# lms-org/trajectory_controller

Measured on AMD Instinct MI355X. Metric: MPC QP solves/sec (horizon N=20, 2 inputs) at 1/2/4/8 MI355X; max|du| vs dlib, higher is better.
Workload: dtype f64; 1 GPU; batch 262144 trajectories per GPU, N=20, 2 inputs, compact (mpcControllerTobi) form, cold start, eps 0.01, max_iter 10000; global_batch=262144, horizon=20, algo=lane_fma, parallelism=batch-sharded x1, batches_in_flight=1, gather=none (1 GPU)

## Files before the change

### trajectory_controller_amd/capi.py

```python
from __future__ import annotations

import ctypes as C
import os

_HERE = os.path.dirname(os.path.abspath(__file__))
LIB_PATH = os.environ.get("TPC_MPC_LIB") or os.path.join(_HERE, "lib", "libtpc_mpc.so")

OK = 0
F64, F32 = 0, 1
HOST, DEVICE = 0, 1
ALGO_AUTO, ALGO_WAVE, ALGO_LANE, ALGO_LANE_FMA, ALGO_GROUP = 0, 1, 2, 3, 4
OPT_WAVE_GROUP, OPT_MAILBOX_HOST, OPT_GROUP_LANES, OPT_HOST_SOLVE_ONE = 1, 2, 3, 4
DEVICE_NONE = -1
FLAG_NONFINITE, FLAG_MAX_ITER, FLAG_BAD_MODEL, FLAG_NOT_POLISHED = 0x1, 0x2, 0x4, 0x8
NEWTON_FALLBACK_SOLVE, NEWTON_FALLBACK_NONE = 0, 1
NEWTON_FALLBACKS = {"solve": NEWTON_FALLBACK_SOLVE, "none": NEWTON_FALLBACK_NONE}
LOOP_RECORD, LOOP_POLISHED, LOOP_NEWTON = 0, 1, 2
PARAM_FAST_CAPPED = 0x1

STATUS_NAMES = {0: "OK", 1: "BAD_ARG", 2: "BAD_WEIGHTS", 3: "BAD_BOUNDS", 4: "BAD_HORIZON",
                5: "BAD_EPS", 6: "NO_DEVICE", 7: "HIP", 8: "ALLOC", 9: "COMM"}
ABI_VERSION = 5
COMM_ID_BYTES = 128

# ... 99 lines not shown
            f"(python -c 'import __graft_entry__ as g; g.build()' or make -C trajectory_controller_amd/csrc)")
    try:
        import torch
    except ImportError:
        pass
    lib = C.CDLL(path)
    vp, i32p, u32p = C.c_void_p, C.POINTER(C.c_int32), C.POINTER(C.c_uint32)
    lib.tpc_mpc_abi_version.restype = C.c_int
    lib.tpc_mpc_supported_horizons.argtypes = [C.POINTER(C.c_int), C.c_int]
    lib.tpc_mpc_default_params.argtypes = [C.POINTER(Params), C.c_int]
    lib.tpc_mpc_create.argtypes = [C.c_int, C.POINTER(vp)]
    lib.tpc_mpc_destroy.argtypes = [vp]
    lib.tpc_mpc_last_error.argtypes = [vp]
    lib.tpc_mpc_last_error.restype = C.c_char_p
    lib.tpc_mpc_solve_one.argtypes = [vp, C.POINTER(Params), C.c_double, C.c_double, C.c_double,
                                      C.POINTER(C.c_double), C.POINTER(C.c_double)]
    lib.tpc_mpc_last_flags.argtypes = [vp, u32p, i32p]
    lib.tpc_mpc_solve_batch_compact.argtypes = [vp, C.POINTER(Params), C.c_int64, vp, vp, vp, vp, vp,
                                                vp, u32p, C.c_int, vp]
    lib.tpc_mpc_solve_batch_general.argtypes = [vp, C.POINTER(Params), C.POINTER(GeneralIO), u32p,
                                                C.c_int, vp]
    lib.tpc_mpc_solve_batch_general_backward.argtypes = [vp, C.POINTER(Params), C.POINTER(GeneralIO),
                                                         C.POINTER(GeneralGrad), u32p, C.c_int, vp]
    lib.tpc_mpc_polish_batch_general.argtypes = [vp, C.POINTER(Params), C.POINTER(GeneralIO), C.POINTER(Polish), u32p,
                                                 C.c_int, vp]
    lib.tpc_mpc_solve_batch_general_sharded.argtypes = [vp, C.POINTER(Params), C.POINTER(GeneralIO), u32p, vp]
    lib.tpc_mpc_rollout.argtypes = [vp, C.POINTER(Params), C.POINTER(GeneralIO), C.c_int32, vp, vp, vp,
                                    vp, u32p, C.c_int, vp]
    lib.tpc_mpc_rollout_record.argtypes = [vp, C.POINTER(Params), C.POINTER(GeneralIO), C.c_int32, vp, vp, vp,
                                           vp, vp, u32p, C.c_int, vp]
    lib.tpc_mpc_rollout_polished.argtypes = [vp, C.POINTER(Params), C.POINTER(GeneralIO), C.c_int32, vp,
                                             C.POINTER(Polish), vp, vp, vp, vp, u32p, C.c_int, vp]
    lib.tpc_mpc_rollout_newton.argtypes = [vp, C.POINTER(Params), C.POINTER(GeneralIO), C.c_int32, vp,
                                           C.POINTER(Polish), C.c_int32, vp, vp, vp, vp, vp, u32p, C.c_int, vp]
    lib.tpc_mpc_rollout_backward.argtypes = [vp, C.POINTER(Params), C.POINTER(GeneralIO), C.c_int32, vp,
                                             C.POINTER(RolloutGrad), u32p, C.c_int, vp]
    lib.tpc_mpc_solve_batch_general_forward.argtypes = [vp, C.POINTER(Params), C.POINTER(GeneralIO), vp,
                                                        C.POINTER(Tangents), vp, u32p, C.c_int, vp]
    lib.tpc_mpc_rollout_forward.argtypes = [vp, C.POINTER(Params), C.POINTER(GeneralIO), C.c_int32, vp, vp, vp,
                                            C.POINTER(Tangents), vp, vp, u32p, C.c_int, vp]
    lib.tpc_mpc_rollout_plant.argtypes = [vp, C.POINTER(Params), C.POINTER(GeneralIO), C.POINTER(Plant), C.c_int32,
                                          C.c_int32, vp, C.POINTER(Polish), C.c_int32, vp, vp, vp, vp, vp, u32p,
                                          C.c_int, vp]
    lib.tpc_mpc_rollout_plant_backward.argtypes = [vp, C.POINTER(Params), C.POINTER(GeneralIO), C.POINTER(Plant),
                                                   C.c_int32, vp, C.POINTER(RolloutGrad), C.POINTER(PlantGrad), u32p,
                                                   C.c_int, vp]
    lib.tpc_mpc_rollout_plant_forward.argtypes = [vp, C.POINTER(Params), C.POINTER(GeneralIO), C.POINTER(Plant),
                                                  C.c_int32, vp, vp, vp, C.POINTER(Tangents),
                                                  C.POINTER(PlantTangents), vp, vp, u32p, C.c_int, vp]
    lib.tpc_mpc_set_profiling.argtypes = [vp, C.c_int]
    lib.tpc_mpc_last_kernel_times.argtypes = [vp, C.POINTER(C.c_double), C.POINTER(C.c_double),
                                              C.POINTER(C.c_int)]
    lib.tpc_mpc_follow_batch.argtypes = [vp, C.POINTER(Params), C.POINTER(Trajectories), vp, vp, C.c_int32,
                                         vp, vp, vp, vp, vp, u32p, vp]
    lib.tpc_mpc_last_lane_stats.argtypes = [vp, C.POINTER(C.c_uint64), C.POINTER(C.c_uint64)]
    lib.tpc_mpc_x_set_work_hint.argtypes = [vp, vp, C.c_int64, C.c_int]
    lib.tpc_mpc_set_option.argtypes = [vp, C.c_int, C.c_int64]
    lib.tpc_mpc_x_set_group_share.argtypes = [vp, C.c_int, C.c_int]
    lib.tpc_mpc_x_set_lanex_below.argtypes = [vp, C.c_int64]
    lib.tpc_mpc_x_set_queue_key.argtypes = [vp, C.c_int]
    lib.tpc_mpc_x_last_queue_key.argtypes = [vp, C.POINTER(C.c_int)]
    lib.tpc_mpc_x_queue_key_predict.argtypes = [vp, vp, vp, C.c_int64, vp]
    lib.tpc_mpc_gather_shards.argtypes = [vp, C.c_int64, C.POINTER(C.c_void_p), C.c_int, C.c_int, vp]
    lib.tpc_mpc_reserve.argtypes = [vp, C.POINTER(Params), C.c_int64, C.c_int]
    lib.tpc_mpc_build_info.restype = C.c_char_p
    lib.tpc_mpc_set_resident.argtypes = [vp, C.c_int64]
    lib.tpc_mpc_solve_batch_compact_mixed.argtypes = [vp, C.POINTER(Params), C.c_int64, vp, vp, vp, vp, vp, vp,
                                                      vp, u32p, C.c_int, vp]
    lib.tpc_mpc_follow_batch_horizon.argtypes = [vp, C.POINTER(Params), C.POINTER(Trajectories), vp, vp, vp,
                                                 C.c_int32, vp, vp, vp, vp, vp, vp, u32p, vp]
    lib.tpc_mpc_comm_unique_id.argtypes = [vp, C.c_size_t]
    lib.tpc_mpc_comm_init_rank.argtypes = [vp, vp, C.c_size_t, C.c_int, C.c_int]
    lib.tpc_mpc_comm_test_mode.argtypes = [vp, C.c_int, C.c_int]
    lib.tpc_mpc_comm_destroy.argtypes = [vp]
    lib.tpc_mpc_shard_range.argtypes = [C.c_int64, C.c_int, C.c_int, C.POINTER(C.c_int64), C.POINTER(C.c_int64)]
    lib.tpc_mpc_solve_batch_compact_sharded.argtypes = [vp, C.POINTER(Params), C.c_int64, vp, vp, vp, vp, vp, vp,
                                                        u32p, vp]
    i64p = C.POINTER(C.c_int64)
    lib.tpc_mpc_shard_map.argtypes = [C.c_int64, C.c_int, C.c_int, C.c_int, i64p, i64p, i64p]
    lib.tpc_mpc_solve_batch_compact_sharded_split.argtypes = [vp, C.POINTER(Params), C.c_int64, C.c_int, vp, vp, vp, vp, vp, vp,
                                                              u32p, vp]
    lib.tpc_mpc_gather_shards_split.argtypes = [vp, C.c_int64, C.c_int, C.POINTER(C.c_void_p), C.c_int, C.c_int, vp]
    lib.tpc_mpc_x_exchange_plan.argtypes = [C.c_int64, C.c_int, C.c_int, C.c_int, C.c_int, i64p, C.c_int, i64p]
    for name in EXPORTS:
        getattr(lib, name)
    if path == LIB_PATH:
        _lib = lib
    return lib


def default_params(horizon: int, dtype: int = F64, algo: int = ALGO_AUTO, **overrides) -> Params:
    lib = load_library()
    p = Params()
    rc = lib.tpc_mpc_default_params(C.byref(p), horizon)
    if rc != OK:
        raise TpcMpcError(rc, f"unsupported horizon {horizon}")
    p.dtype, p.algo = dtype, algo
    for k, val in overrides.items():
        if k in ("lower", "upper"):
            getattr(p, k)[0], getattr(p, k)[1] = float(val[0]), float(val[1])
        else:
            setattr(p, k, val)
    return p
```

### trajectory_controller_amd/csrc/mpc_internal.h

```cpp
#pragma once

#include <hip/hip_runtime.h>
#include <stdint.h>

namespace tpc {

constexpr int kWave = 64;

struct Knobs {
    double eps;
    uint32_t max_iter;
    uint32_t smo_iters;
};

struct CompactArgs {
    int64_t n;
    const void *v, *dy, *dphi;
    void *front, *rear;
    int32_t* iters;
    uint32_t* flags;
    const int32_t* work_hint;
    double step, wheelbase;
    double q[2], r[2], lo[2], hi[2];
    int table_key;
};

constexpr int kQueueKeyLambda = 0, kQueueKeyTableUsed = 1, kQueueKeyHint = 2;

struct OneArgs {
    double v, dy, dphi;
    double step, wheelbase;
    double q[2], r[2], lo[2], hi[2];
    uint64_t* out;
    uint64_t* info;
    static constexpr int32_t* iters = nullptr;
    static constexpr uint32_t* flags = nullptr;
};

struct GeneralArgs {
    int64_t n, ld;
    const void *A, *B, *C, *Q, *R, *lo, *hi, *x0, *targets;
    void *controls, *v;
    void* u0;
    int32_t* iters;
    uint32_t* flags;
    const int32_t* work_hint;
    int shift_controls;
};

struct Workspace {
    void* state;
    uint32_t* ticket;
    unsigned long long* stats;
    int64_t capacity_bytes;
    uint32_t *keys, *rank, *order;
    void* sort_temp;
    size_t sort_temp_bytes;
    hipEvent_t* ev;
    int wave_group = 0;
    int group_lanes = 0;
    int max_waves = 0;
    bool group_pair = false;
    int64_t lanex_below = -1;
    int cu_count = 0;
};

constexpr int kQueueTickets = 16;
constexpr int kQueueTicketStride = 64;
constexpr int64_t kQueueTicketBytes = (int64_t)kQueueTickets * kQueueTicketStride * 4;
constexpr int64_t kWaveQueueMaxInstances = 32768;

constexpr int kAlgoMixed = 101;
constexpr int kAlgoGeneric = 100;
constexpr int kMaxHorizon = 64;
int64_t generic_scratch_bytes(int H, int dtype, int64_t n);
hipError_t generic_compact(int dtype, int H, const CompactArgs& a, const Knobs& k, void* scratch, hipStream_t s);
hipError_t generic_general(int dtype, int I, int H, const GeneralArgs& a, const Knobs& k, void* scratch, hipStream_t s);

size_t sort_temp_bytes(int64_t n);
hipError_t order_begin(void* temp, hipStream_t s);
hipError_t presolve_merge(const uint32_t* queue, const uint32_t* queue_len, int64_t n, const void* sf, const void* sr,
                          const int32_t* si, void* f, void* r, int32_t* it, uint32_t limit, hipStream_t s);
hipError_t presolve_merge_rows(const uint32_t* queue, const uint32_t* queue_len, int64_t n, const void* su, const int32_t* si,
                               void* u, int32_t* it, int rows, int64_t ld, uint32_t limit, hipStream_t s);
const uint32_t* order_queue_len(const void* temp);
hipError_t order_finish(const uint32_t* keys, const uint32_t* rank, uint32_t* order, int64_t n, void* temp,
                        hipStream_t s);

struct RolloutStepArgs {
    int64_t n, ld, ld_out, ld_nlt;
    int I, H, step, steps;
    const void *A, *B, *C;
    void* x;
    void* targets;
    const void* controls;
    const void* new_last_targets;
    void* controls_out;
    void* states_out;
    const int32_t* iters_step;
    int32_t* iters_out;
    void* sequences_out;
    const void* disturbance;
    int64_t ld_d;
};
hipError_t launch_rollout_step(int dtype, const RolloutStepArgs& a, hipStream_t s);

struct FollowArgs {
    int64_t n, ld;
    int max_points;
    const float *px, *py, *dx, *dy, *vel;
    const int32_t* count;
    const float* car_velocity;
    const float* look_ahead;
    const float *lut_x, *lut_y;
    int lut_n;
    double *v_out, *ysoll_out, *phisoll_out;
    float *target_speed, *target_distance;
};
hipError_t launch_traj_point(const FollowArgs& a, hipStream_t s);
struct FollowHorizonArgs {
    int H;
    int64_t ldw;
    const float* step_spacing;
    double step, wheelbase;
    double q[2], r[2], lo[2], hi[2];
    double *A, *B, *C, *Q, *R, *lo_out, *hi_out, *x0, *targets;
    double* targets_copy;
    int64_t ld_copy;
};
hipError_t launch_traj_horizon(const FollowArgs& a, const FollowHorizonArgs& f, hipStream_t s);
hipError_t launch_follow_post(int64_t n, const float* target_speed, double* front, double* rear, hipStream_t s);

}
```

### trajectory_controller_amd/csrc/mpc_lane_inst.hip

```cpp
#include <cstdint>

#include "mpc_lane.h"
#include "mpc_lanex.h"

#ifndef TPC_LANE_H
#error "compile with -DTPC_LANE_H=<horizon>"
#endif

namespace tpc {

namespace {

constexpr int kH = TPC_LANE_H;

template <class Tag, class Kernel>
inline int pg_grid(Kernel kernel, int block) {
    constexpr int kMaxDev = 64;
    static int cache[kMaxDev] = {0};
    int dev = 0;
    if (hipGetDevice(&dev) != hipSuccess) dev = 0;
    if (dev >= 0 && dev < kMaxDev && cache[dev] > 0) return cache[dev];
    int cus = 256, per_cu = 4;
    hipDeviceProp_t prop;
    if (hipGetDeviceProperties(&prop, dev) == hipSuccess) cus = prop.multiProcessorCount;
    if (hipOccupancyMaxActiveBlocksPerMultiprocessor(&per_cu, kernel, block, 0) != hipSuccess || per_cu < 1)
        per_cu = 1;
    if (per_cu > 4) per_cu = 4;
    if (dev >= 0 && dev < kMaxDev) cache[dev] = cus * per_cu;
    return cus * per_cu;
}
struct TagState {}; struct TagFast {}; struct TagExact {}; struct TagLanex {}; template <int I> struct TagLanexG {};

inline bool wants_state(const CompactArgs&) { return false; }
inline bool wants_state(const GeneralArgs& a) { return a.controls != nullptr || a.v != nullptr; }

template <typename T, int I, class Model, class Args>
hipError_t phase1(const Args& a, const Knobs& k, const Workspace& ws, hipStream_t s) {
    T* recs = (T*)ws.state;
    hipError_t e = hipMemsetAsync(ws.ticket, 0, sizeof(uint32_t), s);
    if (e == hipSuccess) e = hipMemsetAsync(ws.stats, 0, 3 * sizeof(unsigned long long), s);
    if (e == hipSuccess) e = order_begin(ws.sort_temp, s);
    if (e != hipSuccess) return e;
    const int cd_grid = (int)((a.n + kWave - 1) / kWave);
    if (ws.ev) (void)hipEventRecord(ws.ev[0], s);
    hipLaunchKernelGGL((lane_cd_kernel<T, I, kH, Model, Args>), dim3(cd_grid), dim3(kWave), 0, s, a, k, recs,
                       ws.keys, ws.rank, (uint32_t*)ws.sort_temp, ws.stats, wants_state(a) ? 0 : 1);
    e = hipGetLastError();
    if (e != hipSuccess) return e;
    e = order_finish(ws.keys, ws.rank, ws.order, a.n, ws.sort_temp, s);
    if (e != hipSuccess) return e;
    if (ws.ev) (void)hipEventRecord(ws.ev[1], s);
    return hipSuccess;
}
template <typename T, int I, class Model, class Args>
hipError_t phase2(const Args& a, const Knobs& k, const Workspace& ws, hipStream_t s, bool only_if_refused) {
    T* recs = (T*)ws.state;
    if (wants_state(a)) {
        const int grid_cap = pg_grid<TagState>(lane_pg_kernel<T, I, kH, Model, Args>, kWave);
        const int64_t need = (a.n + kWave - 1) / kWave;
        hipLaunchKernelGGL((lane_pg_kernel<T, I, kH, Model, Args>), dim3((unsigned)(need < grid_cap ? need : grid_cap)),
                           dim3(kWave), 0, s, a, k, (const T*)recs, (const uint32_t*)ws.order, ws.ticket, ws.stats,
                           only_if_refused ? 1 : 0);
    } else {
        constexpr int bt = kWave * FusedOcc<T, kH>::value;
        const int64_t need = (a.n + bt - 1) / bt;
        const uint32_t* queue_len = order_queue_len(ws.sort_temp);
        if constexpr (Model::kFastStop) {
            if (!only_if_refused) {
                const int fast_cap = pg_grid<TagFast>(lane_pg_fused_kernel<T, I, kH, Model, Args, true>, bt);
                hipLaunchKernelGGL((lane_pg_fused_kernel<T, I, kH, Model, Args, true>),
                                   dim3((unsigned)(need < fast_cap ? need : fast_cap)), dim3(bt), 0, s, a, k,
                                   (const T*)recs, (const uint32_t*)ws.order, ws.ticket, ws.stats, queue_len);
            }
        }
        const int grid_cap = pg_grid<TagExact>(lane_pg_fused_kernel<T, I, kH, Model, Args, false>, bt);
        hipLaunchKernelGGL((lane_pg_fused_kernel<T, I, kH, Model, Args, false>),
                           dim3((unsigned)(need < grid_cap ? need : grid_cap)), dim3(bt), 0, s, a, k,
                           (const T*)recs, (const uint32_t*)ws.order, ws.ticket, ws.stats, queue_len);
    }
    return hipGetLastError();
}

inline int64_t lanex_below(const Workspace& ws, bool general) {
    if (ws.lanex_below >= 0) return ws.lanex_below;
    const int64_t at = general ? (kH == 40 ? 49152 : (kH == 30 ? 57344 : (kH == 20 ? 81920 : (kH == 10 ? 98304 : 0))))
                               : (kH == 40 ? 60000 : (kH == 30 ? 65536 : (kH == 20 || kH == 10 ? 98304 : 0)));
    const int cus = ws.cu_count > 0 ? ws.cu_count : 256;
    return at * cus / 256 < at ? at * cus / 256 : at;
}

template <typename T, int I, class Model, class Args>
hipError_t run(const Args& a, const Knobs& k, const Workspace& ws, hipStream_t s) {
    if (a.n <= 0) return hipSuccess;
    hipError_t e = phase1<T, I, Model, Args>(a, k, ws, s);
    if (e != hipSuccess) return e;
    if constexpr (std::is_same<Model, CompactModel<T>>::value && sizeof(T) == 8 && LanexPlan<kH>::built) {
        if (a.n < lanex_below(ws, false)) {
            constexpr int ng = LanexPlan<kH>::NG;
            const int64_t need = (a.n + ng - 1) / ng;
            const int grid_cap = pg_grid<TagLanex>(lanex_pg_kernel<T, kH>, kWave);
            hipLaunchKernelGGL((lanex_pg_kernel<T, kH>), dim3((unsigned)(need < grid_cap ? need : grid_cap)), dim3(kWave), 0, s, a, k,
                               (const T*)ws.state, (const uint32_t*)ws.order, ws.ticket, ws.stats, order_queue_len(ws.sort_temp),
                               GroupRefillBatch<LanexPlan<kH>::G>::value);
            e = hipGetLastError();
            if (ws.ev) (void)hipEventRecord(ws.ev[2], s);
            return e;
        }
    }
    if constexpr (std::is_same<Args, GeneralArgs>::value && sizeof(T) == 8 && LanexPlan<kH>::built) {
        if (a.n < lanex_below(ws, true)) {
            constexpr int ng = LanexPlan<kH>::NG;
            const int64_t need = (a.n + ng - 1) / ng;
            if (wants_state(a)) {
                const int grid_cap = pg_grid<TagLanexG<I + 2>>(lanexg_pg_kernel<T, I, kH, true>, kWave);
                hipLaunchKernelGGL((lanexg_pg_kernel<T, I, kH, true>), dim3((unsigned)(need < grid_cap ? need : grid_cap)), dim3(kWave), 0, s,
                                   a, k, (const T*)ws.state, (const uint32_t*)ws.order, ws.ticket, ws.stats, (const uint32_t*)nullptr,
                                   GroupRefillBatch<LanexPlan<kH>::G>::value);
            } else {
                const int grid_cap = pg_grid<TagLanexG<I>>(lanexg_pg_kernel<T, I, kH>, kWave);
                hipLaunchKernelGGL((lanexg_pg_kernel<T, I, kH>), dim3((unsigned)(need < grid_cap ? need : grid_cap)), dim3(kWave), 0, s, a, k,
                                   (const T*)ws.state, (const uint32_t*)ws.order, ws.ticket, ws.stats, order_queue_len(ws.sort_temp),
                                   GroupRefillBatch<LanexPlan<kH>::G>::value);
            }
            e = hipGetLastError();
            if (ws.ev) (void)hipEventRecord(ws.ev[2], s);
            return e;
        }
    }
    e = phase2<T, I, Model, Args>(a, k, ws, s, false);
    if (ws.ev) (void)hipEventRecord(ws.ev[2], s);
    return e;
}

template <typename T, int I, class Model, class Args, int SUBSET = 1>
hipError_t resolve(const Args& a, const Knobs& k, const Workspace& ws, const int32_t* select, const uint32_t* gate, hipStream_t s,
                   double lambda_from = 0.0, const uint32_t* pre_len = nullptr, uint32_t pre_limit = 0u) {
    if (a.n <= 0) return hipSuccess;
    T* recs = (T*)ws.state;
    uint32_t* queue_len = ws.ticket + 1;
    hipError_t e = hipMemsetAsync(ws.ticket, 0, 32, s);
    if (e != hipSuccess) return e;
    const int grid = (int)((a.n + kWave - 1) / kWave);
    hipLaunchKernelGGL((lane_cd_kernel<T, I, kH, Model, Args, SUBSET>), dim3(grid), dim3(kWave), 0, s, a, k, recs, ws.order,
                       (uint32_t*)nullptr, queue_len, ws.stats, 1, select, gate, (T)lambda_from, pre_len, pre_limit);
    if constexpr (std::is_same<Model, CompactModel<T>>::value && sizeof(T) == 8 && LanexPlan<kH>::built) {
        constexpr int ng = LanexPlan<kH>::NG;
        const int64_t need = (a.n + ng - 1) / ng;
        if constexpr (SUBSET == 2) {
            const int64_t solo = (int64_t)pre_limit / ng;
            hipLaunchKernelGGL((lanex_pg_kernel<T, kH, true>), dim3((unsigned)(need < solo ? need : solo)), dim3(kWave), 0, s, a, k,
                               (const T*)recs, (const uint32_t*)ws.order, ws.ticket, ws.stats, (const uint32_t*)queue_len, 1, pre_limit);
            return hipGetLastError();
        }
        const int grid_cap = pg_grid<TagLanex>(lanex_pg_kernel<T, kH>, kWave);
        hipLaunchKernelGGL((lanex_pg_kernel<T, kH>), dim3((unsigned)(need < grid_cap ? need : grid_cap)), dim3(kWave), 0, s, a, k,
                           (const T*)recs, (const uint32_t*)ws.order, ws.ticket, ws.stats, (const uint32_t*)queue_len, 1);
        return hipGetLastError();
    } else if constexpr (std::is_same<Args, GeneralArgs>::value && sizeof(T) == 8 && LanexPlan<kH>::built) {
        constexpr int ng = LanexPlan<kH>::NG;
        const int64_t need = (a.n + ng - 1) / ng;
        if constexpr (SUBSET == 2) {
            const int64_t solo = (int64_t)pre_limit / ng;
            hipLaunchKernelGGL((lanexg_pg_kernel<T, I, kH, false, true>), dim3((unsigned)(need < solo ? need : solo)), dim3(kWave), 0, s,
                               a, k, (const T*)recs, (const uint32_t*)ws.order, ws.ticket, ws.stats, (const uint32_t*)queue_len, 1, pre_limit);
            return hipGetLastError();
        }
        const int grid_cap = pg_grid<TagLanexG<I>>(lanexg_pg_kernel<T, I, kH>, kWave);
        hipLaunchKernelGGL((lanexg_pg_kernel<T, I, kH>), dim3((unsigned)(need < grid_cap ? need : grid_cap)), dim3(kWave), 0, s, a, k,
                           (const T*)recs, (const uint32_t*)ws.order, ws.ticket, ws.stats, (const uint32_t*)queue_len, 1);
        return hipGetLastError();
    } else {
    constexpr int bt = kWave * FusedOcc<T, kH>::value;
    const int64_t need = (a.n + bt - 1) / bt;
    const int grid_cap = pg_grid<TagExact>(lane_pg_fused_kernel<T, I, kH, Model, Args, false>, bt);
    hipLaunchKernelGGL((lane_pg_fused_kernel<T, I, kH, Model, Args, false>), dim3((unsigned)(need < grid_cap ? need : grid_cap)),
                       dim3(bt), 0, s, a, k, (const T*)recs, (const uint32_t*)ws.order, ws.ticket, ws.stats, (const uint32_t*)queue_len);
    return hipGetLastError();
    }
}

}

#define TPC_CAT2(a, b) a##b
#define TPC_CAT(a, b) TPC_CAT2(a, b)

#ifndef TPC_SCHED_NAME
#define TPC_SCHED_NAME "default"
#endif
const char* TPC_CAT(lane_build_h, TPC_LANE_H)() { return "sched=" TPC_SCHED_NAME; }

int64_t TPC_CAT(lane_rec_len_h, TPC_LANE_H)(int dtype) {
    return dtype == 0 ? LaneRec<double, kH>::kLen : LaneRec<float, kH>::kLen;
}

hipError_t TPC_CAT(lane_compact_h, TPC_LANE_H)(int dtype, const CompactArgs& a, const Knobs& k,
                                                 const Workspace& ws, hipStream_t s) {
    if (dtype == 0) return run<double, 2, CompactModel<double>, CompactArgs>(a, k, ws, s);
    return run<float, 2, CompactModel<float>, CompactArgs>(a, k, ws, s);
}

hipError_t TPC_CAT(lane_resolve_compact_h, TPC_LANE_H)(const CompactArgs& a, const Knobs& k, const Workspace& ws,
                                                         const int32_t* select, const uint32_t* gate, hipStream_t s,
                                                         double presolved_from, const uint32_t* pre_len, uint32_t pre_limit) {
    return resolve<double, 2, CompactModel<double>, CompactArgs>(a, k, ws, select, gate, s, presolved_from, pre_len, pre_limit);
}
hipError_t TPC_CAT(lane_presolve_compact_h, TPC_LANE_H)(const CompactArgs& a, const Knobs& k, const Workspace& ws,
                                                          double lambda_from, uint32_t limit, hipStream_t s) {
    if constexpr (!LanexPlan<kH>::built) return hipErrorInvalidValue;
    return resolve<double, 2, CompactModel<double>, CompactArgs, 2>(a, k, ws, nullptr, nullptr, s, lambda_from, nullptr, limit);
}
hipError_t TPC_CAT(lane_resolve_general_h, TPC_LANE_H)(int I, const GeneralArgs& a, const Knobs& k, const Workspace& ws,
                                                         const int32_t* select, const uint32_t* gate, hipStream_t s,
                                                         double presolved_from, const uint32_t* pre_len, uint32_t pre_limit) {
    if (I == 2) return resolve<double, 2, GeneralModel<double, 2>, GeneralArgs>(a, k, ws, select, gate, s, presolved_from, pre_len, pre_limit);
    return resolve<double, 1, GeneralModel<double, 1>, GeneralArgs>(a, k, ws, select, gate, s, presolved_from, pre_len, pre_limit);
}
hipError_t TPC_CAT(lane_presolve_general_h, TPC_LANE_H)(int I, const GeneralArgs& a, const Knobs& k, const Workspace& ws,
                                                          double lambda_from, uint32_t limit, hipStream_t s) {
    if constexpr (!LanexPlan<kH>::built) return hipErrorInvalidValue;
    if (I == 2) return resolve<double, 2, GeneralModel<double, 2>, GeneralArgs, 2>(a, k, ws, nullptr, nullptr, s, lambda_from, nullptr, limit);
    return resolve<double, 1, GeneralModel<double, 1>, GeneralArgs, 2>(a, k, ws, nullptr, nullptr, s, lambda_from, nullptr, limit);
}

// ... 21 lines not shown
```

### trajectory_controller_amd/csrc/mpc_sort.hip

```cpp
#include "mpc_internal.h"

namespace tpc {

namespace {

constexpr int kBins = 1 << 16;

constexpr int kScanBlocks = 64, kScanThreads = 256, kPerThread = kBins / kScanBlocks / kScanThreads;

__global__ __launch_bounds__(kScanThreads) void scan_sums_kernel(const uint32_t* __restrict__ hist,
                                                                 uint32_t* __restrict__ block_sum) {
    __shared__ uint32_t part[kScanThreads / 64];
    const int t = threadIdx.x;
    const int top = kBins - 1 - (blockIdx.x * kScanThreads + t) * kPerThread;
    uint32_t sum = 0;
    for (int j = 0; j < kPerThread; ++j) sum += hist[top - j];
    for (int off = 32; off > 0; off >>= 1) sum += __shfl_down(sum, off);
    if ((t & 63) == 0) part[t >> 6] = sum;
    __syncthreads();
    if (t == 0) {
        uint32_t tot = 0;
        for (int w = 0; w < kScanThreads / 64; ++w) tot += part[w];
        block_sum[blockIdx.x] = tot;
    }
}

__global__ __launch_bounds__(kScanThreads) void scan_apply_kernel(uint32_t* __restrict__ hist,
                                                                  const uint32_t* __restrict__ block_sum) {
    __shared__ uint32_t part[kScanThreads];
    const int t = threadIdx.x;
    const int top = kBins - 1 - (blockIdx.x * kScanThreads + t) * kPerThread;
    uint32_t c[kPerThread], sum = 0;
    for (int j = 0; j < kPerThread; ++j) { c[j] = hist[top - j]; sum += c[j]; }
    part[t] = sum;
    __syncthreads();
    for (int off = 1; off < kScanThreads; off <<= 1) {
        const uint32_t add = t >= off ? part[t - off] : 0u;
        __syncthreads();
        part[t] += add;
        __syncthreads();
    }
    uint32_t base = part[t] - sum;
    for (int b = 0; b < (int)blockIdx.x; ++b) base += block_sum[b];
    for (int j = 0; j < kPerThread; ++j) {
        hist[top - j] = base;
        base += c[j];
    }
}

__global__ void scatter_kernel(const uint32_t* __restrict__ keys, const uint32_t* __restrict__ rank,
                               const uint32_t* __restrict__ base, uint32_t* __restrict__ order, int64_t n) {
    for (int64_t i = (int64_t)blockIdx.x * blockDim.x + threadIdx.x; i < n; i += (int64_t)gridDim.x * blockDim.x)
        order[base[keys[i] >> 16] + rank[i]] = (uint32_t)i;
}

}

size_t sort_temp_bytes(int64_t) { return (size_t)(kBins + kScanBlocks) * sizeof(uint32_t); }

const uint32_t* order_queue_len(const void* temp) { return (const uint32_t*)temp + 127; }

hipError_t order_begin(void* temp, hipStream_t s) {
    return hipMemsetAsync(temp, 0, (size_t)kBins * sizeof(uint32_t), s);
}

hipError_t order_finish(const uint32_t* keys, const uint32_t* rank, uint32_t* order, int64_t n, void* temp,
                        hipStream_t s) {
    uint32_t* hist = (uint32_t*)temp;
    const int block = 256;
    int64_t g = (n + block - 1) / block;
    const unsigned grid = (unsigned)(g < 2048 ? g : 2048);
    uint32_t* block_sum = hist + kBins;
    hipLaunchKernelGGL(scan_sums_kernel, dim3(kScanBlocks), dim3(kScanThreads), 0, s, (const uint32_t*)hist, block_sum);
    hipLaunchKernelGGL(scan_apply_kernel, dim3(kScanBlocks), dim3(kScanThreads), 0, s, hist, (const uint32_t*)block_sum);
    hipLaunchKernelGGL(scatter_kernel, dim3(grid), dim3(block), 0, s, keys, rank, (const uint32_t*)hist, order, n);
    return hipGetLastError();
}

template <typename T>
__global__ void presolve_merge_kernel(const uint32_t* __restrict__ queue, const uint32_t* __restrict__ queue_len,
                                      const T* __restrict__ sf, const T* __restrict__ sr, const int32_t* __restrict__ si,
                                      T* __restrict__ f, T* __restrict__ r, int32_t* __restrict__ it, uint32_t limit) {
    const uint32_t nq = *queue_len;
    if (nq > limit) return;
    for (uint32_t q = blockIdx.x * blockDim.x + threadIdx.x; q < nq; q += gridDim.x * blockDim.x) {
        const uint32_t k = queue[q];
        f[k] = sf[k];
        r[k] = sr[k];
        if (it) it[k] = si[k];
    }
}
__global__ void presolve_merge_rows_kernel(const uint32_t* __restrict__ queue, const uint32_t* __restrict__ queue_len,
                                           const double* __restrict__ su, const int32_t* __restrict__ si, double* __restrict__ u,
                                           int32_t* __restrict__ it, int rows, int64_t ld, uint32_t limit) {
    const uint32_t nq = *queue_len;
    if (nq > limit) return;
    for (uint32_t q = blockIdx.x * blockDim.x + threadIdx.x; q < nq; q += gridDim.x * blockDim.x) {
        const uint32_t k = queue[q];
        for (int j = 0; j < rows; ++j) u[(int64_t)j * ld + k] = su[(int64_t)j * ld + k];
        if (it) it[k] = si[k];
    }
}
hipError_t presolve_merge_rows(const uint32_t* queue, const uint32_t* queue_len, int64_t n, const void* su, const int32_t* si,
                               void* u, int32_t* it, int rows, int64_t ld, uint32_t limit, hipStream_t s) {
    const int64_t blocks = (n + 255) / 256;
    hipLaunchKernelGGL(presolve_merge_rows_kernel, dim3((unsigned)(blocks < 256 ? blocks : 256)), dim3(256), 0, s, queue, queue_len,
                       (const double*)su, si, (double*)u, it, rows, ld, limit);
    return hipGetLastError();
}
hipError_t presolve_merge(const uint32_t* queue, const uint32_t* queue_len, int64_t n, const void* sf, const void* sr,
                          const int32_t* si, void* f, void* r, int32_t* it, uint32_t limit, hipStream_t s) {
    const int64_t blocks = (n + 255) / 256;
    hipLaunchKernelGGL(presolve_merge_kernel<double>, dim3((unsigned)(blocks < 256 ? blocks : 256)), dim3(256), 0, s, queue, queue_len,
                       (const double*)sf, (const double*)sr, si, (double*)f, (double*)r, it, limit);
    return hipGetLastError();
}

}
```

### trajectory_controller_amd/csrc/mpc_ub_inst.hip

```cpp
#include <cstdint>
#include <type_traits>

#include "mpc_ub.h"

#ifndef TPC_UB_H
#error "compile with -DTPC_UB_H=<horizon>"
#endif

namespace tpc {

hipError_t ub_pg_asm_launch(const CompactArgs& a, const Knobs& k, const Workspace& ws, int64_t need, hipStream_t s);
hipError_t ub_pg_asm_launch_h10(const CompactArgs& a, const Knobs& k, const Workspace& ws, int64_t need, hipStream_t s);

namespace {

constexpr int kH = TPC_UB_H;

template <class Tag, class Kernel>
inline int ub_grid(Kernel kernel, int block) {
    constexpr int kMaxDev = 64;
    static int cache[kMaxDev] = {0};
    int dev = 0;
    if (hipGetDevice(&dev) != hipSuccess) dev = 0;
    if (dev >= 0 && dev < kMaxDev && cache[dev] > 0) return cache[dev];
    int cus = 256, per_cu = 4;
    hipDeviceProp_t prop;
    if (hipGetDeviceProperties(&prop, dev) == hipSuccess) cus = prop.multiProcessorCount;
    if (hipOccupancyMaxActiveBlocksPerMultiprocessor(&per_cu, kernel, block, 0) != hipSuccess || per_cu < 1)
        per_cu = 1;
    if (per_cu > 4) per_cu = 4;
    if (dev >= 0 && dev < kMaxDev) cache[dev] = cus * per_cu;
    return cus * per_cu;
}
template <typename T, bool EQB, int MODE> struct TagPg {};

template <typename T, bool EQB>
hipError_t phase1(const CompactArgs& a, const Knobs& k, const Workspace& ws, hipStream_t s) {
    T* recs = (T*)ws.state;
    hipError_t e = hipMemsetAsync(ws.ticket, 0, sizeof(uint32_t), s);
    if (e == hipSuccess) e = hipMemsetAsync(ws.stats, 0, 3 * sizeof(unsigned long long), s);
    if (e == hipSuccess) e = order_begin(ws.sort_temp, s);
    if (e != hipSuccess) return e;
    const int cd_grid = (int)((a.n + kWave - 1) / kWave);
    if (ws.ev) (void)hipEventRecord(ws.ev[0], s);
    hipLaunchKernelGGL((ub_cd_kernel<T, kH, EQB>), dim3(cd_grid), dim3(kWave), 0, s, a, k, recs, ws.keys, ws.rank,
                       (uint32_t*)ws.sort_temp, ws.stats);
    e = hipGetLastError();
    if (e != hipSuccess) return e;
    e = order_finish(ws.keys, ws.rank, ws.order, a.n, ws.sort_temp, s);
    if (e != hipSuccess) return e;
    if (ws.ev) (void)hipEventRecord(ws.ev[1], s);
    return hipSuccess;
}
template <typename T, bool EQB, int MODE>
hipError_t pg_launch(const CompactArgs& a, const Knobs& k, const Workspace& ws, hipStream_t s) {
    constexpr int bt = kWave * UbPlan<T, kH>::occ;
    const int64_t need = (a.n + bt - 1) / bt;
#if (TPC_UB_H == 20 || TPC_UB_H == 10) && !defined(TPC_UB_NO_ASM)
    if constexpr (sizeof(T) == 8 && EQB && MODE == 2) {
        const int64_t waves = (a.n + kWave - 1) / kWave;
        return kH == 20 ? ub_pg_asm_launch(a, k, ws, waves, s) : ub_pg_asm_launch_h10(a, k, ws, waves, s);
    }
#endif
    int cap = ub_grid<TagPg<T, EQB, MODE>>(ub_pg_kernel<T, kH, EQB, MODE>, bt);
    if (ws.max_waves > 0 && cap > ws.max_waves / UbPlan<T, kH>::occ) cap = ws.max_waves / UbPlan<T, kH>::occ;
    hipLaunchKernelGGL((ub_pg_kernel<T, kH, EQB, MODE>), dim3((unsigned)(need < cap ? need : cap)), dim3(bt), 0, s, a, k,
                       (const T*)ws.state, (const uint32_t*)ws.order, ws.ticket, ws.stats, order_queue_len(ws.sort_temp));
    return hipGetLastError();
}

template <typename T, bool EQB>
hipError_t run(const CompactArgs& a, const Knobs& k, const Workspace& ws, hipStream_t s) {
    if (a.n <= 0) return hipSuccess;
    hipError_t e = phase1<T, EQB>(a, k, ws, s);
    if (e != hipSuccess) return e;
    e = pg_launch<T, EQB, 2>(a, k, ws, s);
    if constexpr (sizeof(T) == 4) {
        if (e == hipSuccess) e = pg_launch<T, EQB, 1>(a, k, ws, s);
    }
    if (e == hipSuccess) e = pg_launch<T, EQB, 0>(a, k, ws, s);
    if (ws.ev) (void)hipEventRecord(ws.ev[2], s);
    return e;
}

}

#define TPC_CAT2(a, b) a##b
#define TPC_CAT(a, b) TPC_CAT2(a, b)

hipError_t TPC_CAT(ub_compact_h, TPC_UB_H)(int dtype, int equal_bounds, const CompactArgs& a, const Knobs& k,
                                            const Workspace& ws, hipStream_t s) {
    if (dtype == 0) {
        if constexpr (kH >= 30) return hipErrorInvalidValue;
        else return equal_bounds ? run<double, true>(a, k, ws, s) : run<double, false>(a, k, ws, s);
    }
    return run<float, true>(a, k, ws, s);
}

hipError_t TPC_CAT(ub_phase1_h, TPC_UB_H)(int dtype, int equal_bounds, const CompactArgs& a, const Knobs& k,
                                           const Workspace& ws, hipStream_t s) {
    if (dtype == 0) return equal_bounds ? phase1<double, true>(a, k, ws, s) : phase1<double, false>(a, k, ws, s);
    return phase1<float, true>(a, k, ws, s);
}
hipError_t TPC_CAT(ub_exact_h, TPC_UB_H)(int dtype, int equal_bounds, const CompactArgs& a, const Knobs& k,
                                          const Workspace& ws, hipStream_t s) {
    if (dtype == 0) return equal_bounds ? pg_launch<double, true, 0>(a, k, ws, s) : pg_launch<double, false, 0>(a, k, ws, s);
    return pg_launch<float, true, 0>(a, k, ws, s);
}

}
```

### trajectory_controller_amd/csrc/mpc_ubg_inst.hip

```cpp
#include <cstdint>
#include <type_traits>

#include "mpc_ubg.h"

#ifndef TPC_UBG_H
#error "compile with -DTPC_UBG_H=<horizon>"
#endif

namespace tpc {

namespace {

constexpr int kH = TPC_UBG_H;

template <class Tag, class Kernel>
inline int ubg_grid(Kernel kernel, int block) {
    constexpr int kMaxDev = 64;
    static int cache[kMaxDev] = {0};
    int dev = 0;
    if (hipGetDevice(&dev) != hipSuccess) dev = 0;
    if (dev >= 0 && dev < kMaxDev && cache[dev] > 0) return cache[dev];
    int cus = 256, per_cu = 4;
    hipDeviceProp_t prop;
    if (hipGetDeviceProperties(&prop, dev) == hipSuccess) cus = prop.multiProcessorCount;
    if (hipOccupancyMaxActiveBlocksPerMultiprocessor(&per_cu, kernel, block, 0) != hipSuccess || per_cu < 1)
        per_cu = 1;
    if (per_cu > 4) per_cu = 4;
    if (dev >= 0 && dev < kMaxDev) cache[dev] = cus * per_cu;
    return cus * per_cu;
}
template <typename T, int I> struct TagFast {};
template <typename T, int I> struct TagExact {};

template <typename T, int I>
hipError_t phase1(const GeneralArgs& a, const Knobs& k, const Workspace& ws, hipStream_t s) {
    T* recs = (T*)ws.state;
    hipError_t e = hipMemsetAsync(ws.ticket, 0, sizeof(uint32_t), s);
    if (e == hipSuccess) e = hipMemsetAsync(ws.stats, 0, 3 * sizeof(unsigned long long), s);
    if (e == hipSuccess) e = order_begin(ws.sort_temp, s);
    if (e != hipSuccess) return e;
    const int cd_grid = (int)((a.n + kWave - 1) / kWave);
    if (ws.ev) (void)hipEventRecord(ws.ev[0], s);
    hipLaunchKernelGGL((ubg_cd_kernel<T, I, kH>), dim3(cd_grid), dim3(kWave), 0, s, a, k, recs, ws.keys, ws.rank,
                       (uint32_t*)ws.sort_temp, ws.stats);
    e = hipGetLastError();
    if (e != hipSuccess) return e;
    e = order_finish(ws.keys, ws.rank, ws.order, a.n, ws.sort_temp, s);
    if (e != hipSuccess) return e;
    if (ws.ev) (void)hipEventRecord(ws.ev[1], s);
    return hipSuccess;
}
template <typename T, int I, bool FAST>
hipError_t pg_launch(const GeneralArgs& a, const Knobs& k, const Workspace& ws, hipStream_t s) {
    constexpr int bt = kWave * UbgPlan<T, kH>::occ;
    const int64_t need = (a.n + bt - 1) / bt;
    const int cap = ubg_grid<std::conditional_t<FAST, TagFast<T, I>, TagExact<T, I>>>(ubg_pg_kernel<T, I, kH, FAST>, bt);
    hipLaunchKernelGGL((ubg_pg_kernel<T, I, kH, FAST>), dim3((unsigned)(need < cap ? need : cap)), dim3(bt), 0, s, a, k,
                       (const T*)ws.state, (const uint32_t*)ws.order, ws.ticket, ws.stats, order_queue_len(ws.sort_temp));
    return hipGetLastError();
}

template <typename T, int I>
hipError_t run(const GeneralArgs& a, const Knobs& k, const Workspace& ws, hipStream_t s) {
    if (a.n <= 0) return hipSuccess;
    if (a.controls || a.v) return hipErrorInvalidValue;
    hipError_t e = phase1<T, I>(a, k, ws, s);
    if (e != hipSuccess) return e;
    e = pg_launch<T, I, true>(a, k, ws, s);
    if (e == hipSuccess) e = pg_launch<T, I, false>(a, k, ws, s);
    if (ws.ev) (void)hipEventRecord(ws.ev[2], s);
    return e;
}

}

#define TPC_CAT2(a, b) a##b
#define TPC_CAT(a, b) TPC_CAT2(a, b)

hipError_t TPC_CAT(ub_general_h, TPC_UBG_H)(int dtype, int inputs, const GeneralArgs& a, const Knobs& k,
                                             const Workspace& ws, hipStream_t s) {
    if (inputs != 1 && inputs != 2) return hipErrorInvalidValue;
    if (dtype == 0) return inputs == 1 ? run<double, 1>(a, k, ws, s) : run<double, 2>(a, k, ws, s);
    return inputs == 1 ? run<float, 1>(a, k, ws, s) : run<float, 2>(a, k, ws, s);
}

hipError_t TPC_CAT(ubg_phase1_h, TPC_UBG_H)(int dtype, int inputs, const GeneralArgs& a, const Knobs& k, const Workspace& ws, hipStream_t s) {
    if (dtype == 0) return inputs == 1 ? phase1<double, 1>(a, k, ws, s) : phase1<double, 2>(a, k, ws, s);
    return inputs == 1 ? phase1<float, 1>(a, k, ws, s) : phase1<float, 2>(a, k, ws, s);
}
hipError_t TPC_CAT(ubg_exact_h, TPC_UBG_H)(int dtype, int inputs, const GeneralArgs& a, const Knobs& k, const Workspace& ws, hipStream_t s) {
    if (dtype == 0) return inputs == 1 ? pg_launch<double, 1, false>(a, k, ws, s) : pg_launch<double, 2, false>(a, k, ws, s);
    return inputs == 1 ? pg_launch<float, 1, false>(a, k, ws, s) : pg_launch<float, 2, false>(a, k, ws, s);
}

}
```

### trajectory_controller_amd/csrc/tpc_mpc_api.cpp

```cpp
#include "tpc_mpc_context.h"
#include "tpc_mpc_experimental.h"
#include "auto_table.h"
#include "mpc_queue_key_table.h"
#include "mpc_grad_model.h"
#include "mpc_polish_model.h"
#include "mpc_rollout_newton.h"
#include "mpc_tangent_model.h"

#include <cmath>
#include <cstdlib>
#include <mutex>
#include <vector>

namespace tpc {
#define TPC_DECL_H(h)                                                                             \
    hipError_t lane_compact_h##h(int, const CompactArgs&, const Knobs&, const Workspace&, hipStream_t); \
    hipError_t lane_general_h##h(int, int, const GeneralArgs&, const Knobs&, const Workspace&, hipStream_t); \
    hipError_t lane_resolve_compact_h##h(const CompactArgs&, const Knobs&, const Workspace&, const int32_t*, const uint32_t*, hipStream_t, double, const uint32_t*, uint32_t); \
    hipError_t lane_presolve_compact_h##h(const CompactArgs&, const Knobs&, const Workspace&, double, uint32_t, hipStream_t); \
    hipError_t lane_resolve_general_h##h(int, const GeneralArgs&, const Knobs&, const Workspace&, const int32_t*, const uint32_t*, hipStream_t, double, const uint32_t*, uint32_t); \
    hipError_t lane_presolve_general_h##h(int, const GeneralArgs&, const Knobs&, const Workspace&, double, uint32_t, hipStream_t); \
    hipError_t wave_compact_h##h(int, const CompactArgs&, const Knobs&, const Workspace&, hipStream_t); \
    hipError_t wave_general_h##h(int, int, const GeneralArgs&, const Knobs&, const Workspace&, hipStream_t); \
    hipError_t ub_compact_h##h(int, int, const CompactArgs&, const Knobs&, const Workspace&, hipStream_t); \
// ... 206 lines not shown
                                                       : wave_compact_h##h(dtype, a, k, ws, s);
        X(4) X(5) X(10) X(20) X(30) X(40)
#undef X
    }
    return hipErrorInvalidValue;
}
hipError_t dispatch_general(int algo, int I, int H, int dtype, const GeneralArgs& a, const Knobs& k,
                            const Workspace& ws, hipStream_t s) {
    if (algo == kAlgoGeneric) return generic_launch(ws, s, [&] { return generic_general(dtype, I, H, a, k, ws.state, s); });
    if (algo == TPC_MPC_ALGO_GROUP) {
        switch (H) {
#define X(h) case h: return groupg_general_h##h(dtype, I, ws.group_lanes, a, k, ws, s);
            X(10) X(20) X(30) X(40)
#undef X
        }
        return hipErrorInvalidValue;
    }
    if (algo == TPC_MPC_ALGO_LANE_FMA) {
        switch (H) {
#define X(h) case h: return ub_general_h##h(dtype, I, a, k, ws, s);
            X(4) X(5) X(10) X(20)
#undef X
        }
        return hipErrorInvalidValue;
    }
    switch (H) {
#define X(h) case h: return algo == TPC_MPC_ALGO_LANE ? lane_general_h##h(dtype, I, a, k, ws, s) \
                                                       : wave_general_h##h(dtype, I, a, k, ws, s);
        X(4) X(5) X(10) X(20) X(30) X(40)
#undef X
    }
    return hipErrorInvalidValue;
}

bool wants_cap_resolve(const tpc_mpc_params* p, int algo_ran) {
    return p->algo == TPC_MPC_ALGO_AUTO && p->dtype == TPC_MPC_F64 && p->max_iter > 0 &&
           (p->options & TPC_MPC_PARAM_FAST_CAPPED) == 0 && horizon_specialised(p->horizon) &&
           (algo_ran == TPC_MPC_ALGO_WAVE || algo_ran == TPC_MPC_ALGO_LANE_FMA || algo_ran == TPC_MPC_ALGO_GROUP);
}
int cap_iters_buffer(tpc_mpc_context* h, int64_t n, int32_t** out) {
    int rc = ensure(h, &h->cap_iters, &h->cap_iters_bytes, pad256(n * 4));
    if (rc) return rc;
    *out = (int32_t*)h->cap_iters;
    return TPC_MPC_OK;
}
hipError_t resolve_compact(int H, const CompactArgs& a, const Knobs& k, const Workspace& ws, hipStream_t s, double presolved_from = 0.0,
                           const uint32_t* pre_len = nullptr, uint32_t pre_limit = 0u) {
    switch (H) {
#define X(h) case h: return lane_resolve_compact_h##h(a, k, ws, a.iters, a.flags, s, presolved_from, pre_len, pre_limit);
        X(4) X(5) X(10) X(20) X(30) X(40)
#undef X
    }
    return hipErrorInvalidValue;
}
hipError_t resolve_general(int I, int H, const GeneralArgs& a, const Knobs& k, const Workspace& ws, hipStream_t s,
                           double presolved_from = 0.0, const uint32_t* pre_len = nullptr, uint32_t pre_limit = 0u) {
    switch (H) {
#define X(h) case h: return lane_resolve_general_h##h(I, a, k, ws, a.iters, a.flags, s, presolved_from, pre_len, pre_limit);
        X(4) X(5) X(10) X(20) X(30) X(40)
#undef X
    }
    return hipErrorInvalidValue;
}

int prepare_workspace(tpc_mpc_context* h, int algo, int H, int dtype, int64_t n, Workspace* ws, int form = 0) {
    ws->state = nullptr;
    ws->ticket = h->ws_words;
    ws->stats = (unsigned long long*)(h->ws_words + 4);
    ws->capacity_bytes = 0;
    ws->ev = h->profiling ? h->ev : nullptr;
    ws->wave_group = h->opt_wave_group;
    ws->group_lanes = group_lanes(h, H, dtype, n, form);
    ws->max_waves = h->max_waves;
    if (h->pre_busy && h->pre_group_waves > 0 && (ws->max_waves == 0 || ws->max_waves > h->pre_group_waves))
        ws->max_waves = h->pre_group_waves;
    ws->group_pair = group_pair(h, H, dtype, n, form);
    ws->lanex_below = h->opt_lanex_below;
    ws->cu_count = h->cu_count;
    h->ev_valid = h->profiling;
    h->last_algo = algo;
    ws->keys = ws->rank = ws->order = nullptr;
    ws->sort_temp = nullptr;
    ws->sort_temp_bytes = 0;
    if (algo == kAlgoGeneric) {
        int rc = ensure(h, &h->ws_state, &h->ws_bytes, pad256(generic_scratch_bytes(H, dtype, n)));
        if (rc) return rc;
        ws->state = h->ws_state;
        ws->capacity_bytes = h->ws_bytes;
    }
    if (algo == TPC_MPC_ALGO_WAVE) {
        int rc = ensure(h, &h->ws_state, &h->ws_bytes, pad256(n * 4) + kQueueTicketBytes);
        if (rc) return rc;
        ws->order = (uint32_t*)h->ws_state;
        ws->ticket = (uint32_t*)((char*)h->ws_state + pad256(n * 4));
        ws->capacity_bytes = h->ws_bytes;
    }
    if (algo == TPC_MPC_ALGO_LANE || algo == TPC_MPC_ALGO_LANE_FMA || algo == TPC_MPC_ALGO_GROUP) {
        const int64_t rec_b = pad256(lane_rec_len(H, dtype) * (int64_t)esize(dtype) * n);
        const int64_t col_b = pad256(n * 4);
        const size_t tmp_b = sort_temp_bytes(n);
        int rc = ensure(h, &h->ws_state, &h->ws_bytes, rec_b + 3 * col_b + pad256((int64_t)tmp_b));
        if (rc) return rc;
        char* b = (char*)h->ws_state;
        ws->state = b;
        ws->keys = (uint32_t*)(b + rec_b);
        ws->rank = (uint32_t*)(b + rec_b + col_b);
        ws->order = (uint32_t*)(b + rec_b + 2 * col_b);
        ws->sort_temp = b + rec_b + 3 * col_b;
        ws->sort_temp_bytes = tmp_b;
        ws->capacity_bytes = h->ws_bytes;
    }
    return TPC_MPC_OK;
}

int resolve_reserve(tpc_mpc_context* h, int H, int dtype, int64_t n) { return reserve_lane_workspace(h, H, dtype, n); }
int resolve_workspace(tpc_mpc_context* h, int H, int dtype, int64_t n, Workspace* ws) {
    const bool ev_valid = h->ev_valid;
    const int last_algo = h->last_algo;
    const int rc = prepare_workspace(h, TPC_MPC_ALGO_LANE, H, dtype, n, ws);
    h->ev_valid = ev_valid;
    h->last_algo = last_algo;
    ws->ev = nullptr;
    ws->ticket = h->ws_words + 16;
    ws->stats = (unsigned long long*)(h->ws_words + 18);
    return rc;
}

hipError_t copy_rows(void* dst, int64_t dpitch, const void* src, int64_t spitch, int64_t width, int64_t rows,
                     hipMemcpyKind kind, hipStream_t s) {
    if (rows <= 0 || width <= 0) return hipSuccess;
    if (dpitch == width && spitch == width) return hipMemcpyAsync(dst, src, (size_t)(width * rows), kind, s);
    return hipMemcpy2DAsync(dst, (size_t)dpitch, src, (size_t)spitch, (size_t)width, (size_t)rows, kind, s);
}

int check_general_io(tpc_mpc_context* h, const tpc_mpc_general_io* io, int mem) {
    if (!io) return fail(h, TPC_MPC_ERR_BAD_ARG, "null io");
    if (io->inputs != 1 && io->inputs != 2) return fail(h, TPC_MPC_ERR_BAD_ARG, "inputs must be 1 or 2");
    if (io->n < 0 || io->ld < io->n || io->n > 0x7fffffffll)
        return fail(h, TPC_MPC_ERR_BAD_ARG, "need 0 <= n <= ld, n < 2^31");
    if (mem != TPC_MPC_HOST && mem != TPC_MPC_DEVICE) return fail(h, TPC_MPC_ERR_BAD_ARG, "bad memory kind");
    return TPC_MPC_OK;
}

}

namespace tpc {

bool group_applicable(const tpc_mpc_context* h, const tpc_mpc_params* p, int H) {
    return (p->algo == TPC_MPC_ALGO_AUTO || p->algo == TPC_MPC_ALGO_GROUP) && fma_usable(p) && group_lanes(h, H) > 0;
}

int check_common(tpc_mpc_context* h, const tpc_mpc_params* p, bool host_ok) {
    if (!h) return fail(nullptr, TPC_MPC_ERR_BAD_ARG, "null handle");
    if (h->host_only && !host_ok)
        return fail(h, TPC_MPC_ERR_NO_DEVICE, "host-only handle (TPC_MPC_DEVICE_NONE): only tpc_mpc_solve_one is served");
    if (!p) return fail(h, TPC_MPC_ERR_BAD_ARG, "null params");
    if (!horizon_ok(p->horizon))
        return fail(h, TPC_MPC_ERR_BAD_HORIZON, "horizon %d outside 1 .. %d", p->horizon, kMaxHorizon);
    if (p->dtype != TPC_MPC_F64 && p->dtype != TPC_MPC_F32) return fail(h, TPC_MPC_ERR_BAD_ARG, "bad dtype");
    if (p->algo < TPC_MPC_ALGO_AUTO || p->algo > TPC_MPC_ALGO_GROUP) return fail(h, TPC_MPC_ERR_BAD_ARG, "bad algo");
    if (!(p->eps > 0)) return fail(h, TPC_MPC_ERR_BAD_EPS, "eps must be > 0 (mpc.h:202)");
    if (p->options & ~TPC_MPC_PARAM_FAST_CAPPED) return fail(h, TPC_MPC_ERR_BAD_ARG, "unknown bits in tpc_mpc_params.options");
    if (p->max_iter > 0x7fffffffull || p->smo_iters > 0x7fffffffull)
        return fail(h, TPC_MPC_ERR_BAD_ARG, "max_iter / smo_iters must fit in 31 bits");
    return TPC_MPC_OK;
}

int check_compact_model(tpc_mpc_context* h, const tpc_mpc_params* p) {
    if (!(p->weight_y >= 0) || !(p->weight_phi >= 0))
        return fail(h, TPC_MPC_ERR_BAD_WEIGHTS, "min(Q) >= 0 violated (mpc_abstract.h:90-97)");
    if (!(p->weight_steering_front > 0) || !(p->weight_steering_rear > 0))
        return fail(h, TPC_MPC_ERR_BAD_WEIGHTS, "min(R) > 0 violated (mpc_abstract.h:90-97)");
    for (int j = 0; j < 2; ++j)
        if (!(p->upper[j] >= p->lower[j]))
            return fail(h, TPC_MPC_ERR_BAD_BOUNDS, "upper >= lower violated (mpc_abstract.h:90-97)");
    if (!std::isfinite(p->step_size) || !std::isfinite(p->wheelbase) || p->wheelbase == 0)
        return fail(h, TPC_MPC_ERR_BAD_ARG, "step_size / wheelbase must be finite, wheelbase != 0");
    return TPC_MPC_OK;
}

int stream_order_begin(tpc_mpc_context* h, hipStream_t s) {
    if (h->have_last && h->last_stream != s) HIP_TRY(h, hipStreamWaitEvent(s, h->done_ev, 0));
    return TPC_MPC_OK;
}
int stream_order_end(tpc_mpc_context* h, hipStream_t s) {
    HIP_TRY(h, hipEventRecord(h->done_ev, s));
    h->last_stream = s;
    h->have_last = true;
    return TPC_MPC_OK;
}

int finish_flags(tpc_mpc_context* h, uint32_t* flags_out, hipStream_t s) {
    if (!flags_out) return TPC_MPC_OK;
    uint32_t f = 0;
    HIP_TRY(h, hipMemcpyAsync(&f, h->ws_words + 1, sizeof(f), hipMemcpyDeviceToHost, s));
    HIP_TRY(h, hipStreamSynchronize(s));
    *flags_out = f;
    return TPC_MPC_OK;
}

int reserve_lane_workspace(tpc_mpc_context* h, int H, int dtype, int64_t n) {
    const bool ev_valid = h->ev_valid;
    const int last_algo = h->last_algo;
    Workspace ws;
    const int rc = prepare_workspace(h, horizon_specialised(H) ? TPC_MPC_ALGO_LANE : kAlgoGeneric, H, dtype, n, &ws);
    h->ev_valid = ev_valid;
    h->last_algo = last_algo;
    return rc;
}

int context_new(int device, int cu_count, tpc_mpc_context** out) {
    tpc_mpc_context* h = new (std::nothrow) tpc_mpc_context;
    if (!h) return fail(nullptr, TPC_MPC_ERR_ALLOC, "out of host memory");
    h->device = device;
    h->cu_count = cu_count;
    h->device_cu_count = cu_count;
    hipError_t e = hipSetDevice(device);
    if (e == hipSuccess) e = hipMalloc((void**)&h->ws_words, 128);
    if (e == hipSuccess) e = hipMemset(h->ws_words, 0, 128);
    if (e == hipSuccess) e = hipHostMalloc(&h->pin_host, 512, hipHostMallocMapped | hipHostMallocCoherent);
    if (e == hipSuccess) e = hipHostGetDevicePointer(&h->pin_dev, h->pin_host, 0);
    if (e == hipSuccess) e = hipEventCreateWithFlags(&h->done_ev, hipEventDisableTiming);
    if (e != hipSuccess) {
        (void)tpc_mpc_destroy(h);
        return fail(nullptr, TPC_MPC_ERR_HIP, "create: %s", hipGetErrorString(e));
    }
    std::memset(h->pin_host, 0, 512);
    *out = h;
    return TPC_MPC_OK;
}

static double presolve_lambda(const tpc_mpc_params* p);
static int presolve_scratch(tpc_mpc_context* h, int H, int dtype, int64_t n, int64_t side_bytes, Workspace* ws, char** side) {
    const int64_t rec_b = pad256(lane_rec_len(H, dtype) * (int64_t)esize(dtype) * n), col_b = pad256(n * 4);
    const size_t tmp_b = sort_temp_bytes(n);
    const int64_t lane_b = rec_b + 3 * col_b + pad256((int64_t)tmp_b);
    int rc = ensure(h, &h->pre, &h->pre_bytes, lane_b + side_bytes);
    if (rc) return rc;
    if (!h->pre_stream) HIP_TRY(h, hipStreamCreateWithFlags(&h->pre_stream, hipStreamNonBlocking));
    if (!h->pre_fork) HIP_TRY(h, hipEventCreateWithFlags(&h->pre_fork, hipEventDisableTiming));
    if (!h->pre_done) HIP_TRY(h, hipEventCreateWithFlags(&h->pre_done, hipEventDisableTiming));
    char* b = (char*)h->pre;
    std::memset(ws, 0, sizeof(*ws));
    ws->state = b;
    ws->keys = (uint32_t*)(b + rec_b);
    ws->rank = (uint32_t*)(b + rec_b + col_b);
    ws->order = (uint32_t*)(b + rec_b + 2 * col_b);
    ws->sort_temp = b + rec_b + 3 * col_b;
    ws->sort_temp_bytes = tmp_b;
    ws->capacity_bytes = lane_b;
    ws->ev = nullptr;
    ws->lanex_below = h->opt_lanex_below;
    ws->cu_count = h->cu_count;
    ws->ticket = h->ws_words + 24;
    ws->stats = (unsigned long long*)(h->ws_words + 26);
    *side = b + lane_b;
    return TPC_MPC_OK;
}
static bool presolve_share(tpc_mpc_context* h, int64_t n, Presolve* ps) {
    const int simds = (h->device_cu_count > 0 ? h->device_cu_count : 256) * 4;
    const int solo_waves = simds * 7 / 16;
    if (n > (int64_t)solo_waves * 8 * 5) return false;
    ps->limit = (uint32_t)solo_waves * 8u;
    ps->group_waves = simds - solo_waves;
    return true;
}

int general_launch(tpc_mpc_context* h, const tpc_mpc_params* p, const tpc_mpc_general_io* io, hipStream_t s) {
    const int I = io->inputs, H = p->horizon;
    const int64_t n = io->n;
    const int algo = pick_algo(h, p->algo, I, H, n, p->dtype, fma_general_usable(H, io->controls_inout, io->v_inout), false,
                                   group_general_usable(p->dtype, H, io->controls_inout, io->v_inout));
    if (algo < 0) return fail(h, TPC_MPC_ERR_BAD_HORIZON, "the WAVE kernel exists for the specialised horizons with inputs*horizon <= 64 only; use LANE or AUTO");
    GeneralArgs a;
    std::memset(&a, 0, sizeof(a));
    a.n = n; a.ld = io->ld; a.shift_controls = 1;
    a.A = io->A; a.B = io->B; a.C = io->C; a.Q = io->Q; a.R = io->R; a.lo = io->lower; a.hi = io->upper;
    a.x0 = io->x0; a.targets = io->targets; a.controls = io->controls_inout; a.v = io->v_inout;
    a.u0 = io->u0; a.iters = io->iters;
    a.flags = h->ws_words + 1;
    a.work_hint = take_hint(h, n);
    const bool fix = wants_cap_resolve(p, algo) && !a.controls && !a.v;
    int rc = TPC_MPC_OK;
    if (fix && !a.iters) rc = cap_iters_buffer(h, n, &a.iters);
    if (!rc && fix) rc = resolve_reserve(h, H, p->dtype, n);
    if (rc) return rc;
    Presolve ps;
    const double lf = presolve_lambda(p);
    const int64_t ubytes = pad256((int64_t)I * a.ld * 8);
    if (fix && algo == TPC_MPC_ALGO_GROUP && lf > 0.0 && !h->pre_busy && presolve_share(h, n, &ps)) {
        Workspace wp;
        char* side = nullptr;
        rc = presolve_scratch(h, H, p->dtype, n, ubytes + pad256(n * 4), &wp, &side);
        if (rc) return rc;
        GeneralArgs a2 = a;
        a2.u0 = side;
        a2.iters = (int32_t*)(side + ubytes);
        a2.work_hint = nullptr;
        ps.side_front = side;
        ps.side_iters = a2.iters;
        ps.queue = wp.order;
        ps.queue_len = wp.ticket + 1;
        ps.lambda_from = lf;
        HIP_TRY(h, hipEventRecord(h->pre_fork, s));
        HIP_TRY(h, hipStreamWaitEvent(h->pre_stream, h->pre_fork, 0));
        ps.on = true;
        h->pre_busy = true;
        h->pre_group_waves = ps.group_waves;
        hipError_t e = hipErrorInvalidValue;
        switch (H) {
#define X(hh) case hh: e = lane_presolve_general_h##hh(I, a2, knobs_of(p), wp, lf, ps.limit, h->pre_stream); break;
            X(4) X(5) X(10) X(20) X(30) X(40)
#undef X
        }
        if (e != hipSuccess) {
            h->pre_busy = false;
            (void)hipEventRecord(h->pre_done, h->pre_stream);
            (void)hipStreamWaitEvent(s, h->pre_done, 0);
            return hip_fail(h, e, "kernel launch (presolve)");
        }
    }
    auto join = [&]() {
        if (!ps.on) return;
        ps.on = false;
        h->pre_busy = false;
        (void)hipEventRecord(h->pre_done, h->pre_stream);
        (void)hipStreamWaitEvent(s, h->pre_done, 0);
    };
    Workspace ws;
    rc = prepare_workspace(h, algo, H, p->dtype, n, &ws, 1);
    if (rc) { join(); return rc; }
    hipError_t e = dispatch_general(algo, I, H, p->dtype, a, knobs_of(p), ws, s);
    join();
    if (e == hipSuccess && ps.lambda_from > 0.0)
        e = presolve_merge_rows(ps.queue, ps.queue_len, n, ps.side_front, ps.side_iters, a.u0, a.iters, I, a.ld, ps.limit, s);
    if (e == hipSuccess && fix) {
        Workspace ws2;
        rc = resolve_workspace(h, H, p->dtype, n, &ws2);
// ... 265 lines not shown
        *out = nullptr;
        if (device == TPC_MPC_DEVICE_NONE) {
            tpc_mpc_context* h = new (std::nothrow) tpc_mpc_context;
            if (!h) return fail(nullptr, TPC_MPC_ERR_ALLOC, "out of host memory");
            h->device = -1;
            h->host_only = true;
            *out = h;
            return TPC_MPC_OK;
        }
        int count = 0;
        hipError_t e = hipGetDeviceCount(&count);
        if (e != hipSuccess || count <= 0)
            return fail(nullptr, TPC_MPC_ERR_NO_DEVICE, "no HIP device: %s",
                        e != hipSuccess ? hipGetErrorString(e) : "count == 0");
        if (device < 0 || device >= count) return fail(nullptr, TPC_MPC_ERR_NO_DEVICE, "device index out of range");
        hipDeviceProp_t prop;
        e = hipGetDeviceProperties(&prop, device);
        if (e != hipSuccess) return fail(nullptr, TPC_MPC_ERR_NO_DEVICE, "%s", hipGetErrorString(e));
        if (std::strncmp(prop.gcnArchName, "gfx950", 6) != 0)
            return fail(nullptr, TPC_MPC_ERR_NO_DEVICE, "device is %s, this library carries gfx950 code only",
                        prop.gcnArchName);
        return context_new(device, prop.multiProcessorCount, out);
    });
}

int tpc_mpc_destroy(tpc_mpc_handle h) {
    if (!h) return TPC_MPC_OK;
    return guarded(nullptr, [&]() -> int {
        if (h->host_only) { delete h; return TPC_MPC_OK; }
        (void)hipSetDevice(h->device);
        one_shot_destroy(h);
        comm_destroy(h);
        for (int i = 0; i < tpc_mpc_context::kMaxKids; ++i) {
            if (h->kid_stream[i]) { (void)hipStreamSynchronize(h->kid_stream[i]); (void)hipStreamDestroy(h->kid_stream[i]); }
            if (h->kid_done[i]) (void)hipEventDestroy(h->kid_done[i]);
            if (h->kids[i]) (void)tpc_mpc_destroy(h->kids[i]);
        }
        if (h->fork_ev) (void)hipEventDestroy(h->fork_ev);
        if (h->ws_state) (void)hipFree(h->ws_state);
        if (h->ws_words) (void)hipFree(h->ws_words);
        if (h->stage) (void)hipFree(h->stage);
        if (h->roll) (void)hipFree(h->roll);
        if (h->cap_iters) (void)hipFree(h->cap_iters);
        if (h->grad_ws) (void)hipFree(h->grad_ws);
        if (h->newton) (void)hipFree(h->newton);
        if (h->newton_fb) (void)hipFree(h->newton_fb);
        if (h->mix) (void)hipFree(h->mix);
        if (h->gather) (void)hipFree(h->gather);
        if (h->pre_stream) { (void)hipStreamSynchronize(h->pre_stream); (void)hipStreamDestroy(h->pre_stream); }
        if (h->pre_fork) (void)hipEventDestroy(h->pre_fork);
        if (h->pre_done) (void)hipEventDestroy(h->pre_done);
        if (h->pre) (void)hipFree(h->pre);
        if (h->hint_own) (void)hipFree(h->hint_own);
        if (h->pin_host) (void)hipHostFree(h->pin_host);
        if (h->done_ev) (void)hipEventDestroy(h->done_ev);
        for (auto& e : h->ev) if (e) (void)hipEventDestroy(e);
        delete h;
        return TPC_MPC_OK;
    });
}

const char* tpc_mpc_last_error(tpc_mpc_handle h) { return h ? h->err : g_create_error; }

int tpc_mpc_solve_batch_compact(tpc_mpc_handle h, const tpc_mpc_params* p, int64_t n, const void* v,
                                const void* delta_y, const void* delta_phi, void* steering_front,
                                void* steering_rear, int32_t* iters, uint32_t* flags_out, int mem,
                                void* stream) {
    return guarded(h, [&]() -> int {
        int rc = check_common(h, p);
        if (rc) return rc;
        rc = check_compact_model(h, p);
        if (rc) return rc;
        if (n < 0 || n > 0x7fffffffll) return fail(h, TPC_MPC_ERR_BAD_ARG, "need 0 <= n < 2^31");
        if (mem != TPC_MPC_HOST && mem != TPC_MPC_DEVICE) return fail(h, TPC_MPC_ERR_BAD_ARG, "bad memory kind");
        if (n == 0) { if (flags_out) *flags_out = 0; return TPC_MPC_OK; }
        if (!v || !delta_y || !delta_phi || !steering_front || !steering_rear)
            return fail(h, TPC_MPC_ERR_BAD_ARG, "null batch pointer");
        HIP_TRY(h, hipSetDevice(h->device));
        hipStream_t s = (hipStream_t)stream;
        const int64_t es = (int64_t)esize(p->dtype);
        StreamOrderScope order(h, s);
        rc = order.begin();
        if (rc) return rc;
        HIP_TRY(h, hipMemsetAsync(h->ws_words + 1, 0, sizeof(uint32_t), s));
        if (mem == TPC_MPC_DEVICE) {
            rc = compact_launch(h, p, n, v, delta_y, delta_phi, steering_front, steering_rear, iters, s);
            if (rc) return rc;
        } else {
            const int64_t col = pad256(n * es), icol = pad256(n * 4);
            rc = ensure(h, &h->stage, &h->stage_bytes, 5 * col + icol);
            if (rc) return rc;
            char* b = (char*)h->stage;
            HIP_TRY(h, hipMemcpyAsync(b, v, n * es, hipMemcpyHostToDevice, s));
            HIP_TRY(h, hipMemcpyAsync(b + col, delta_y, n * es, hipMemcpyHostToDevice, s));
            HIP_TRY(h, hipMemcpyAsync(b + 2 * col, delta_phi, n * es, hipMemcpyHostToDevice, s));
            int32_t* d_it = iters ? (int32_t*)(b + 5 * col) : nullptr;
            rc = compact_launch(h, p, n, b, b + col, b + 2 * col, b + 3 * col, b + 4 * col, d_it, s);
            if (rc) return rc;
            HIP_TRY(h, hipMemcpyAsync(steering_front, b + 3 * col, n * es, hipMemcpyDeviceToHost, s));
            HIP_TRY(h, hipMemcpyAsync(steering_rear, b + 4 * col, n * es, hipMemcpyDeviceToHost, s));
            if (iters) HIP_TRY(h, hipMemcpyAsync(iters, d_it, n * 4, hipMemcpyDeviceToHost, s));
            HIP_TRY(h, hipStreamSynchronize(s));
        }
        rc = order.end();
        if (rc) return rc;
        return finish_flags(h, flags_out, s);
    });
}

int tpc_mpc_solve_one(tpc_mpc_handle h, const tpc_mpc_params* p, double v, double delta_y,
                      double delta_phi, double* steering_front, double* steering_rear) {
    return guarded(h, [&]() -> int {
        if (!h) return fail(nullptr, TPC_MPC_ERR_BAD_ARG, "null handle");
        if (!steering_front || !steering_rear) return fail(h, TPC_MPC_ERR_BAD_ARG, "null output pointer");
        int rc = check_common(h, p, true);
        if (rc) return rc;
        rc = check_compact_model(h, p);
        if (rc) return rc;
        if (h->host_only || p->horizon <= h->opt_host_horizon) {
            const bool takes = p->dtype == TPC_MPC_F64 && (p->algo == TPC_MPC_ALGO_AUTO || p->algo == TPC_MPC_ALGO_LANE_FMA) &&
                               fma_usable(p) && horizon_specialised(p->horizon) && host_path_usable();
            if (takes) {
                int iters = 0;
                unsigned flags = 0;
                if (host_solve_one(p, v, delta_y, delta_phi, steering_front, steering_rear, &iters, &flags) == 0) {
                    h->one_flags = flags;
                    h->one_iters = iters;
                    h->one_valid = true;
                    if ((flags & TPC_MPC_FLAG_MAX_ITER) && !h->host_only && p->algo == TPC_MPC_ALGO_AUTO && p->max_iter > 0 &&
                        (p->options & TPC_MPC_PARAM_FAST_CAPPED) == 0) {
                        tpc_mpc_params q = *p;
                        q.algo = TPC_MPC_ALGO_LANE;
                        return one_shot_solve(h, &q, v, delta_y, delta_phi, steering_front, steering_rear);
                    }
                    return TPC_MPC_OK;
                }
            }
            if (h->host_only)
                return fail(h, TPC_MPC_ERR_NO_DEVICE, "host-only handle: the host path takes fp64, AUTO or LANE_FMA, horizons 4 5 10 20 30 40, "
                                                      "finite bounds with upper > lower, on a CPU with fused multiply-add");
        }
        return one_shot_solve(h, p, v, delta_y, delta_phi, steering_front, steering_rear);
    });
}

int tpc_mpc_last_flags(tpc_mpc_handle h, uint32_t* flags, int32_t* iters) {
    return guarded(h, [&]() -> int {
        if (!h) return fail(nullptr, TPC_MPC_ERR_BAD_ARG, "null handle");
        if (!h->one_valid) return fail(h, TPC_MPC_ERR_BAD_ARG, "no tpc_mpc_solve_one on this handle yet");
        if (flags) *flags = h->one_flags;
        if (iters) *iters = h->one_iters;
        return TPC_MPC_OK;
    });
}

int tpc_mpc_solve_batch_general(tpc_mpc_handle h, const tpc_mpc_params* p,
                                const tpc_mpc_general_io* io, uint32_t* flags_out, int mem,
                                void* stream) {
    return guarded(h, [&]() -> int {
        int rc = check_common(h, p);
        if (rc) return rc;
        rc = check_general_io(h, io, mem);
        if (rc) return rc;
        if (io->n == 0) { if (flags_out) *flags_out = 0; return TPC_MPC_OK; }
        if (!io->A || !io->B || !io->C || !io->Q || !io->R || !io->lower || !io->upper || !io->x0 ||
            !io->targets || !io->u0)
            return fail(h, TPC_MPC_ERR_BAD_ARG, "null batch pointer");
        HIP_TRY(h, hipSetDevice(h->device));
        hipStream_t s = (hipStream_t)stream;
        const int64_t es = (int64_t)esize(p->dtype);
        const int I = io->inputs, H = p->horizon;
        const int64_t n = io->n;
        const int algo = pick_algo(h, p->algo, I, H, n, p->dtype, fma_general_usable(H, io->controls_inout, io->v_inout), false,
                                   group_general_usable(p->dtype, H, io->controls_inout, io->v_inout));
        if (algo < 0) return fail(h, TPC_MPC_ERR_BAD_HORIZON, "the WAVE kernel exists for the specialised horizons with inputs*horizon <= 64 only; use LANE or AUTO");
        StreamOrderScope order(h, s);
        rc = order.begin();
        if (rc) return rc;

        GeneralArgs a;
        std::memset(&a, 0, sizeof(a));
        a.n = n;
        a.shift_controls = 1;
        const int64_t lds = (n + 63) / 64 * 64;
        const int comps[12] = {4, 2 * I, 2, 2, I, I, I, 2, 2 * H, H * I, H * I, I};
        int64_t off[13] = {0};
        char* b = nullptr;
        if (mem == TPC_MPC_DEVICE) {
            a.ld = io->ld;
            a.A = io->A; a.B = io->B; a.C = io->C; a.Q = io->Q; a.R = io->R; a.lo = io->lower; a.hi = io->upper;
            a.x0 = io->x0; a.targets = io->targets; a.controls = io->controls_inout; a.v = io->v_inout;
            a.u0 = io->u0; a.iters = io->iters;
        } else {
            const void* src[12] = {io->A, io->B, io->C, io->Q, io->R, io->lower, io->upper, io->x0, io->targets,
                                   io->controls_inout, io->v_inout, nullptr};
            int64_t total = 0;
            for (int c = 0; c < 12; ++c) { off[c] = total; total += pad256((int64_t)comps[c] * lds * es); }
            off[12] = total;
            total += pad256(n * 4);
            rc = ensure(h, &h->stage, &h->stage_bytes, total);
            if (rc) return rc;
            b = (char*)h->stage;
            for (int c = 0; c < 11; ++c)
                if (src[c])
                    HIP_TRY(h, copy_rows(b + off[c], lds * es, src[c], io->ld * es, n * es, comps[c],
                                         hipMemcpyHostToDevice, s));
            a.ld = lds;
            a.A = b + off[0]; a.B = b + off[1]; a.C = b + off[2]; a.Q = b + off[3]; a.R = b + off[4];
            a.lo = b + off[5]; a.hi = b + off[6]; a.x0 = b + off[7]; a.targets = b + off[8];
            a.controls = io->controls_inout ? b + off[9] : nullptr;
            a.v = io->v_inout ? b + off[10] : nullptr;
            a.u0 = b + off[11];
            a.iters = io->iters ? (int32_t*)(b + off[12]) : nullptr;
        }
        a.flags = h->ws_words + 1;
        a.work_hint = take_hint(h, n);
        const bool fix = wants_cap_resolve(p, algo) && !a.controls && !a.v;
        if (fix && !a.iters) {
            rc = cap_iters_buffer(h, n, &a.iters);
            if (rc) return rc;
        }
        if (fix) {
            rc = resolve_reserve(h, H, p->dtype, n);
            if (rc) return rc;
        }

        Workspace ws;
        rc = prepare_workspace(h, algo, H, p->dtype, n, &ws, 1);
        if (rc) return rc;
        HIP_TRY(h, hipMemsetAsync(h->ws_words + 1, 0, sizeof(uint32_t), s));
        hipError_t e = dispatch_general(algo, I, H, p->dtype, a, knobs_of(p), ws, s);
        if (e == hipSuccess && fix) {
            Workspace ws2;
            rc = resolve_workspace(h, H, p->dtype, n, &ws2);
            if (rc) return rc;
            e = resolve_general(I, H, a, knobs_of(p), ws2, s);
        }
        if (e != hipSuccess) return hip_fail(h, e, "kernel launch");
        if (mem == TPC_MPC_HOST) {
            const int64_t hp = io->ld * es, dp = lds * es, w = n * es;
            HIP_TRY(h, copy_rows(io->u0, hp, a.u0, dp, w, I, hipMemcpyDeviceToHost, s));
            if (io->controls_inout)
                HIP_TRY(h, copy_rows(io->controls_inout, hp, a.controls, dp, w, H * I, hipMemcpyDeviceToHost, s));
            if (io->v_inout) HIP_TRY(h, copy_rows(io->v_inout, hp, a.v, dp, w, H * I, hipMemcpyDeviceToHost, s));
            if (io->iters) HIP_TRY(h, hipMemcpyAsync(io->iters, a.iters, n * 4, hipMemcpyDeviceToHost, s));
            HIP_TRY(h, hipStreamSynchronize(s));
        }
        rc = order.end();
        if (rc) return rc;
        return finish_flags(h, flags_out, s);
    });
}

int tpc_mpc_solve_batch_general_backward(tpc_mpc_handle h, const tpc_mpc_params* p, const tpc_mpc_general_io* io,
                                         const tpc_mpc_general_grad* g, uint32_t* flags_out, int mem, void* stream) {
    return guarded(h, [&]() -> int {
        int rc = check_common(h, p, true);
        if (rc) return rc;
        if (p->dtype != TPC_MPC_F64)
            return fail(h, TPC_MPC_ERR_BAD_ARG, "tpc_mpc_solve_batch_general_backward is fp64 only: p->dtype must be TPC_MPC_F64");
        rc = check_general_io(h, io, mem);
        if (rc) return rc;
        if (!g) return fail(h, TPC_MPC_ERR_BAD_ARG, "null gradient struct");
        if (h->host_only && mem == TPC_MPC_DEVICE)
            return fail(h, TPC_MPC_ERR_NO_DEVICE, "host-only handle (TPC_MPC_DEVICE_NONE): the backward pass takes HOST memory only");
        if (io->n == 0) { if (flags_out) *flags_out = 0; return TPC_MPC_OK; }
        if (!io->A || !io->B || !io->C || !io->Q || !io->R || !io->lower || !io->upper || !io->x0 || !io->targets)
            return fail(h, TPC_MPC_ERR_BAD_ARG, "null batch pointer");
        if (!g->controls || !g->grad_controls) return fail(h, TPC_MPC_ERR_BAD_ARG, "null controls / grad_controls");
        const int I = io->inputs, H = p->horizon;
        const int64_t n = io->n;
        const void* src[11] = {io->A, io->B, io->C, io->Q, io->R, io->lower, io->upper, io->x0, io->targets,
                               g->controls, g->grad_controls};
        void* dst[10] = {g->dA, g->dB, g->dC, g->dQ, g->dR, g->dlower, g->dupper, g->dx0, g->dtargets, g->kkt_residual};
        const int comps[21] = {4, 2 * I, 2, 2, I, I, I, 2, 2 * H, H * I, H * I,
                               4, 2 * I, 2, 2, I, I, I, 2, 2 * H, 1};
        auto bind = [](grad::Args* a, const void* const* in, void* const* out) {
            a->A = (const double*)in[0]; a->B = (const double*)in[1]; a->C = (const double*)in[2];
            a->Q = (const double*)in[3]; a->R = (const double*)in[4]; a->lo = (const double*)in[5];
            a->hi = (const double*)in[6]; a->x0 = (const double*)in[7]; a->targets = (const double*)in[8];
            a->u = (const double*)in[9]; a->g = (const double*)in[10];
            a->dA = (double*)out[0]; a->dB = (double*)out[1]; a->dC = (double*)out[2]; a->dQ = (double*)out[3];
            a->dR = (double*)out[4]; a->dlo = (double*)out[5]; a->dhi = (double*)out[6]; a->dx0 = (double*)out[7];
            a->dtargets = (double*)out[8]; a->kkt = (double*)out[9];
        };
        grad::Args a;
        std::memset(&a, 0, sizeof(a));
        a.n = n;
        if (h->host_only) {
            a.ld = io->ld;
            bind(&a, src, dst);
            const uint32_t f = grad_general_host(I, H, a);
            if (flags_out) *flags_out = f;
            return TPC_MPC_OK;
        }
        HIP_TRY(h, hipSetDevice(h->device));
        hipStream_t s = (hipStream_t)stream;
        StreamOrderScope order(h, s);
        rc = order.begin();
        if (rc) return rc;
        rc = ensure(h, &h->grad_ws, &h->grad_ws_bytes, pad256(grad_scratch_bytes(I, H, n)));
        if (rc) return rc;
        const int64_t lds = (n + 63) / 64 * 64;
        int64_t off[21] = {0};
        if (mem == TPC_MPC_DEVICE) {
            a.ld = io->ld;
            bind(&a, src, dst);
        } else {
            int64_t total = 0;
            for (int c = 0; c < 21; ++c) { off[c] = total; total += pad256((int64_t)comps[c] * lds * 8); }
            rc = ensure(h, &h->stage, &h->stage_bytes, total);
            if (rc) return rc;
            char* b = (char*)h->stage;
// ... 177 lines not shown
            else HIP_TRY(h, hipMemsetAsync(w + off[c], 0, (size_t)((int64_t)comps[c] * ldw * es), s));
        }
        const void* d_nlt = new_last_targets;
        int64_t ld_nlt = ld, ld_out = ld;
        char *d_ctrl = (char*)controls_out, *d_states = (char*)states_out, *d_seq = (char*)sequences_out;
        int32_t* d_iters = iters_out;
        int32_t* d_status = polished ? q->status : nullptr;
        char *d_rin = polished ? (char*)q->residual_in : nullptr, *d_rout = polished ? (char*)q->residual_out : nullptr;
        if (host) {
            const int64_t s_nlt = 0, s_ctrl = s_nlt + pad256((int64_t)steps * 2 * ldw * es);
            const int64_t s_states = s_ctrl + pad256((int64_t)steps * I * ldw * es);
            const int64_t s_iters = s_states + pad256((int64_t)steps * 2 * ldw * es);
            const int64_t s_seq = s_iters + pad256((int64_t)steps * ldw * 4);
            const int64_t s_status = s_seq + (sequences_out ? pad256((int64_t)steps * H * I * ldw * es) : 0);
            const int64_t s_rin = s_status + (d_status ? pad256((int64_t)steps * ldw * 4) : 0);
            const int64_t s_rout = s_rin + (d_rin ? pad256((int64_t)steps * ldw * 8) : 0);
            const int64_t s_end = s_rout + (d_rout ? pad256((int64_t)steps * ldw * 8) : 0);
            rc = ensure(h, &h->stage, &h->stage_bytes, s_end);
            if (rc) return rc;
            char* b = (char*)h->stage;
            if (new_last_targets) {
                HIP_TRY(h, copy_rows(b + s_nlt, ldw * es, new_last_targets, ld * es, n * es, (int64_t)steps * 2,
                                     hipMemcpyHostToDevice, s));
                d_nlt = b + s_nlt;
            }
            ld_nlt = ld_out = ldw;
            d_ctrl = b + s_ctrl;
            d_states = states_out ? b + s_states : nullptr;
            d_iters = iters_out ? (int32_t*)(b + s_iters) : nullptr;
            d_seq = sequences_out ? b + s_seq : nullptr;
            if (d_status) d_status = (int32_t*)(b + s_status);
            if (d_rin) d_rin = b + s_rin;
            if (d_rout) d_rout = b + s_rout;
        }

        GeneralArgs a;
        std::memset(&a, 0, sizeof(a));
        a.n = n; a.ld = ldw; a.shift_controls = 1;
        a.A = w + off[0]; a.B = w + off[1]; a.C = w + off[2]; a.Q = w + off[3]; a.R = w + off[4];
        a.lo = w + off[5]; a.hi = w + off[6];
        a.x0 = w + off[7]; a.targets = w + off[8]; a.controls = w + off[9]; a.v = w + off[10]; a.u0 = w + off[11];
        a.iters = (int32_t*)(w + o_iters);
        a.flags = h->ws_words + 1;

        RolloutStepArgs r;
        std::memset(&r, 0, sizeof(r));
        r.n = n; r.ld = ldw; r.ld_out = ld_out; r.ld_nlt = ld_nlt; r.I = I; r.H = H; r.steps = steps;
        r.A = a.A; r.B = a.B; r.C = a.C;
        r.x = w + off[7]; r.targets = w + off[8]; r.controls = w + off[9]; r.new_last_targets = d_nlt;
        r.controls_out = d_ctrl; r.states_out = d_states;
        r.iters_step = a.iters; r.iters_out = d_iters; r.sequences_out = d_seq;
        if (plant_abc) {
            HIP_TRY(h, copy_rows(w + o_pa, ldw * es, plant->A, ld * es, n * es, 4, in_kind, s));
            HIP_TRY(h, copy_rows(w + o_pb, ldw * es, plant->B, ld * es, n * es, 2 * I, in_kind, s));
            HIP_TRY(h, copy_rows(w + o_pc, ldw * es, plant->C, ld * es, n * es, 2, in_kind, s));
            r.A = w + o_pa; r.B = w + o_pb; r.C = w + o_pc;
        }
        if (plant_d) {
            r.disturbance = plant->disturbance; r.ld_d = plant->ld_d;
            if (host) {
                HIP_TRY(h, copy_rows(w + o_pd, ldw * es, plant->disturbance, plant->ld_d * es, n * es, (int64_t)steps * 2,
                                     hipMemcpyHostToDevice, s));
                r.disturbance = w + o_pd; r.ld_d = ldw;
            }
        }

        polish::Args pa;
        std::memset(&pa, 0, sizeof(pa));
        if (polished) {
            pa.n = n; pa.ld = ldw; pa.tol = q->tol; pa.max_rounds = q->max_rounds;
            pa.A = (const double*)a.A; pa.B = (const double*)a.B; pa.C = (const double*)a.C; pa.Q = (const double*)a.Q;
            pa.R = (const double*)a.R; pa.lo = (const double*)a.lo; pa.hi = (const double*)a.hi;
            pa.x0 = (const double*)r.x; pa.targets = (const double*)r.targets; pa.u = (double*)(w + off[9]);
        }

        Workspace ws;
        rc = prepare_workspace(h, algo, H, p->dtype, n, &ws, 1);
        if (rc) return rc;
        HIP_TRY(h, hipMemsetAsync(h->ws_words + 1, 0, sizeof(uint32_t), s));
        const Knobs kn = knobs_of(p);
        for (int st = 0; st < steps; ++st) {
            hipError_t e = dispatch_general(algo, I, H, p->dtype, a, kn, ws, s);
            if (e != hipSuccess) return hip_fail(h, e, "kernel launch");
            r.step = st;
            if (polished) {
                pa.status = d_status ? d_status + (int64_t)st * ld_out : nullptr;
                pa.res_in = d_rin ? (double*)d_rin + (int64_t)st * ld_out : nullptr;
                pa.res_out = d_rout ? (double*)d_rout + (int64_t)st * ld_out : nullptr;
                e = launch_rollout_polish_step(I, pa, r, h->grad_ws, h->ws_words + 1, s);
            } else {
                e = launch_rollout_step(p->dtype, r, s);
            }
            if (e != hipSuccess) return hip_fail(h, e, "rollout step launch");
        }
        if (io->controls_inout)
            HIP_TRY(h, copy_rows(io->controls_inout, ld * es, w + off[9], ldw * es, n * es, H * I, out_kind, s));
        if (io->v_inout) HIP_TRY(h, copy_rows(io->v_inout, ld * es, w + off[10], ldw * es, n * es, H * I, out_kind, s));
        if (host) {
            HIP_TRY(h, copy_rows(controls_out, ld * es, d_ctrl, ldw * es, n * es, (int64_t)steps * I, hipMemcpyDeviceToHost, s));
            if (states_out)
                HIP_TRY(h, copy_rows(states_out, ld * es, d_states, ldw * es, n * es, (int64_t)steps * 2, hipMemcpyDeviceToHost, s));
            if (iters_out)
                HIP_TRY(h, copy_rows(iters_out, ld * 4, d_iters, ldw * 4, n * 4, steps, hipMemcpyDeviceToHost, s));
            if (sequences_out)
                HIP_TRY(h, copy_rows(sequences_out, ld * es, d_seq, ldw * es, n * es, (int64_t)steps * H * I,
                                     hipMemcpyDeviceToHost, s));
            if (d_status)
                HIP_TRY(h, copy_rows(q->status, ld * 4, d_status, ldw * 4, n * 4, steps, hipMemcpyDeviceToHost, s));
            if (d_rin)
                HIP_TRY(h, copy_rows(q->residual_in, ld * 8, d_rin, ldw * 8, n * 8, steps, hipMemcpyDeviceToHost, s));
            if (d_rout)
                HIP_TRY(h, copy_rows(q->residual_out, ld * 8, d_rout, ldw * 8, n * 8, steps, hipMemcpyDeviceToHost, s));
            HIP_TRY(h, hipStreamSynchronize(s));
        }
        rc = order.end();
        if (rc) return rc;
        return finish_flags(h, flags_out, s);
    });
}

}

int tpc_mpc_rollout_polished(tpc_mpc_handle h, const tpc_mpc_params* p, const tpc_mpc_general_io* io,
                             int32_t steps, const void* new_last_targets, const tpc_mpc_polish* q,
                             void* controls_out, void* states_out, int32_t* iters_out, void* sequences_out,
                             uint32_t* flags_out, int mem, void* stream) {
    return rollout_impl(h, p, io, steps, new_last_targets, controls_out, states_out, iters_out, sequences_out, false,
                        true, q, flags_out, mem, stream);
}

int tpc_mpc_rollout(tpc_mpc_handle h, const tpc_mpc_params* p, const tpc_mpc_general_io* io,
                    int32_t steps, const void* new_last_targets, void* controls_out,
                    void* states_out, int32_t* iters_out, uint32_t* flags_out, int mem,
                    void* stream) {
    return rollout_impl(h, p, io, steps, new_last_targets, controls_out, states_out, iters_out, nullptr, false,
                        false, nullptr, flags_out, mem, stream);
}

int tpc_mpc_rollout_record(tpc_mpc_handle h, const tpc_mpc_params* p, const tpc_mpc_general_io* io,
                           int32_t steps, const void* new_last_targets, void* controls_out,
                           void* states_out, int32_t* iters_out, void* sequences_out, uint32_t* flags_out,
                           int mem, void* stream) {
    return rollout_impl(h, p, io, steps, new_last_targets, controls_out, states_out, iters_out, sequences_out, true,
                        false, nullptr, flags_out, mem, stream);
}

static int rollout_newton_impl(tpc_mpc_handle h, const tpc_mpc_params* p, const tpc_mpc_general_io* io, int32_t steps,
                               const void* new_last_targets, const tpc_mpc_polish* q, int32_t fallback,
                               void* controls_out, void* states_out, int32_t* iters_out, void* sequences_out,
                               int32_t* first_unverified, uint32_t* flags_out, int mem, void* stream,
                               const tpc_mpc_plant* plant) {
    return guarded(h, [&]() -> int {
        int rc = check_common(h, p, true);
        if (rc) return rc;
        if (p->dtype != TPC_MPC_F64)
            return fail(h, TPC_MPC_ERR_BAD_ARG, "tpc_mpc_rollout_newton is fp64 only: p->dtype must be TPC_MPC_F64");
        rc = check_general_io(h, io, mem);
        if (rc) return rc;
        if (!q) return fail(h, TPC_MPC_ERR_BAD_ARG, "null polish struct");
        if (!(q->tol > 0.0) || q->max_rounds < 0)
            return fail(h, TPC_MPC_ERR_BAD_ARG, "polish needs tol > 0 and max_rounds >= 0");
        if (fallback != TPC_MPC_NEWTON_FALLBACK_SOLVE && fallback != TPC_MPC_NEWTON_FALLBACK_NONE)
            return fail(h, TPC_MPC_ERR_BAD_ARG, "unknown fallback %d", (int)fallback);
        if (steps < 0 || steps > (1 << 24)) return fail(h, TPC_MPC_ERR_BAD_ARG, "need 0 <= steps <= 2^24");
        const bool solve = fallback == TPC_MPC_NEWTON_FALLBACK_SOLVE;
        if (h->host_only && solve)
// ... 545 lines not shown
                               pl.tC = sep ? (const double*)in[27] : a.t.tC;
                               pl.td = (const double*)in[28];
                               pl.ld_d = staged ? ld : ld_td;
                               if (hf) { *hf = rollout_plant_tangent_host(I, H, a, pl); return hipSuccess; }
                               return rollout_plant_tangent(I, H, a, pl, h->grad_ws, h->ws_words + 1, s);
                           },
                           src_ld);
    });
}

int tpc_mpc_rollout_forward(tpc_mpc_handle h, const tpc_mpc_params* p, const tpc_mpc_general_io* io, int32_t steps,
                            const void* new_last_targets, const void* sequences, const void* states,
                            const tpc_mpc_tangents* t, void* tcontrols, void* tstates, uint32_t* flags_out, int mem,
                            void* stream) {
    return rollout_forward_impl(h, p, io, steps, new_last_targets, sequences, states, t, tcontrols, tstates, flags_out,
                                mem, stream, "tpc_mpc_rollout_forward", false, nullptr, nullptr);
}

int tpc_mpc_rollout_plant_forward(tpc_mpc_handle h, const tpc_mpc_params* p, const tpc_mpc_general_io* io,
                                  const tpc_mpc_plant* plant, int32_t steps, const void* new_last_targets,
                                  const void* sequences, const void* states, const tpc_mpc_tangents* t,
                                  const tpc_mpc_plant_tangents* pt, void* tcontrols, void* tstates,
                                  uint32_t* flags_out, int mem, void* stream) {
    return rollout_forward_impl(h, p, io, steps, new_last_targets, sequences, states, t, tcontrols, tstates, flags_out,
                                mem, stream, "tpc_mpc_rollout_plant_forward", true, plant, pt);
}

namespace {

int check_trajectories(tpc_mpc_context* h, const tpc_mpc_params* p, const tpc_mpc_trajectories* t,
                       const float* lookup_x, const float* lookup_y, int32_t lookup_n) {
    if (p->dtype != TPC_MPC_F64) return fail(h, TPC_MPC_ERR_BAD_ARG, "follow_batch solves in fp64");
    if (!t) return fail(h, TPC_MPC_ERR_BAD_ARG, "null trajectories");
    if (t->n < 0 || t->ld < t->n || t->n > 0x7fffffffll || t->max_points < 0 || lookup_n < 0)
        return fail(h, TPC_MPC_ERR_BAD_ARG, "need 0 <= n <= ld, n < 2^31, max_points >= 0, lookup_n >= 0");
    if (t->n == 0) return TPC_MPC_OK;
    if (!t->pos_x || !t->pos_y || !t->dir_x || !t->dir_y || !t->velocity || !t->count || !t->car_velocity ||
        !t->look_ahead || (lookup_n > 0 && (!lookup_x || !lookup_y)))
        return fail(h, TPC_MPC_ERR_BAD_ARG, "null batch pointer");
    return TPC_MPC_OK;
}

FollowArgs follow_args(const tpc_mpc_trajectories* t, const float* lookup_x, const float* lookup_y, int32_t lookup_n) {
    FollowArgs fa;
    std::memset(&fa, 0, sizeof(fa));
    fa.n = t->n; fa.ld = t->ld; fa.max_points = t->max_points;
    fa.px = t->pos_x; fa.py = t->pos_y; fa.dx = t->dir_x; fa.dy = t->dir_y; fa.vel = t->velocity;
    fa.count = t->count; fa.car_velocity = t->car_velocity; fa.look_ahead = t->look_ahead;
    fa.lut_x = lookup_x; fa.lut_y = lookup_y; fa.lut_n = lookup_n;
    return fa;
}

}

int tpc_mpc_follow_batch(tpc_mpc_handle h, const tpc_mpc_params* p, const tpc_mpc_trajectories* t,
                         const float* lookup_x, const float* lookup_y, int32_t lookup_n,
                         double* steering_front, double* steering_rear, float* target_speed,
                         float* target_distance, int32_t* iters, uint32_t* flags_out, void* stream) {
    return guarded(h, [&]() -> int {
        int rc = check_common(h, p);
        if (rc) return rc;
        rc = check_compact_model(h, p);
        if (rc) return rc;
        rc = check_trajectories(h, p, t, lookup_x, lookup_y, lookup_n);
        if (rc) return rc;
        if (t->n == 0) { if (flags_out) *flags_out = 0; return TPC_MPC_OK; }
        if (!steering_front || !steering_rear || !target_speed || !target_distance)
            return fail(h, TPC_MPC_ERR_BAD_ARG, "null batch pointer");
        HIP_TRY(h, hipSetDevice(h->device));
        hipStream_t s = (hipStream_t)stream;
        const int64_t n = t->n;
        StreamOrderScope order(h, s);
        rc = order.begin();
        if (rc) return rc;
        const int64_t col = pad256(n * 8);
        rc = ensure(h, &h->roll, &h->roll_bytes, 3 * col);
        if (rc) return rc;
        char* b = (char*)h->roll;
        FollowArgs fa = follow_args(t, lookup_x, lookup_y, lookup_n);
        fa.v_out = (double*)b; fa.ysoll_out = (double*)(b + col); fa.phisoll_out = (double*)(b + 2 * col);
        fa.target_speed = target_speed; fa.target_distance = target_distance;
        hipError_t e = launch_traj_point(fa, s);
        if (e != hipSuccess) return hip_fail(h, e, "traj_point launch");
        HIP_TRY(h, hipMemsetAsync(h->ws_words + 1, 0, sizeof(uint32_t), s));
        rc = compact_launch(h, p, n, fa.v_out, fa.ysoll_out, fa.phisoll_out, steering_front, steering_rear, iters, s);
        if (rc) return rc;
        e = launch_follow_post(n, target_speed, steering_front, steering_rear, s);
        if (e != hipSuccess) return hip_fail(h, e, "follow_post launch");
        rc = order.end();
        if (rc) return rc;
        return finish_flags(h, flags_out, s);
    });
}

int tpc_mpc_follow_batch_horizon(tpc_mpc_handle h, const tpc_mpc_params* p, const tpc_mpc_trajectories* t,
                                 const float* step_spacing, const float* lookup_x, const float* lookup_y,
                                 int32_t lookup_n, double* steering_front, double* steering_rear,
                                 float* target_speed, float* target_distance, double* targets_out,
                                 int32_t* iters, uint32_t* flags_out, void* stream) {
    return guarded(h, [&]() -> int {
        int rc = check_common(h, p);
        if (rc) return rc;
        rc = check_compact_model(h, p);
        if (rc) return rc;
        rc = check_trajectories(h, p, t, lookup_x, lookup_y, lookup_n);
        if (rc) return rc;
        if (t->n == 0) { if (flags_out) *flags_out = 0; return TPC_MPC_OK; }
        if (!steering_front || !steering_rear || !target_speed || !target_distance)
            return fail(h, TPC_MPC_ERR_BAD_ARG, "null batch pointer");
        HIP_TRY(h, hipSetDevice(h->device));
        hipStream_t s = (hipStream_t)stream;
        const int64_t n = t->n;
        const int H = p->horizon, I = 2;
        const int algo = pick_algo(h, p->algo, I, H, n, p->dtype, fma_general_usable(H, nullptr, nullptr), false, group_general_usable(p->dtype, H, nullptr, nullptr));
        if (algo < 0) return fail(h, TPC_MPC_ERR_BAD_HORIZON, "the WAVE kernel exists for the specialised horizons with inputs*horizon <= 64 only; use LANE or AUTO");
        StreamOrderScope order(h, s);
        rc = order.begin();
        if (rc) return rc;
        const int64_t ldw = (n + 63) / 64 * 64;
        const int comps[10] = {4, 4, 2, 2, 2, 2, 2, 2, 2 * H, 2};
        int64_t off[10], total = 0;
        for (int c = 0; c < 10; ++c) { off[c] = total; total += pad256((int64_t)comps[c] * ldw * 8); }
        rc = ensure(h, &h->roll, &h->roll_bytes, total);
        if (rc) return rc;
        char* w = (char*)h->roll;
        FollowArgs fa = follow_args(t, lookup_x, lookup_y, lookup_n);
        fa.target_speed = target_speed; fa.target_distance = target_distance;
        FollowHorizonArgs fh;
        std::memset(&fh, 0, sizeof(fh));
        fh.H = H; fh.ldw = ldw; fh.step_spacing = step_spacing;
        fh.step = p->step_size; fh.wheelbase = p->wheelbase;
        fh.q[0] = p->weight_y; fh.q[1] = p->weight_phi;
        fh.r[0] = p->weight_steering_front; fh.r[1] = p->weight_steering_rear;
        for (int j = 0; j < 2; ++j) { fh.lo[j] = p->lower[j]; fh.hi[j] = p->upper[j]; }
        fh.A = (double*)(w + off[0]); fh.B = (double*)(w + off[1]); fh.C = (double*)(w + off[2]);
        fh.Q = (double*)(w + off[3]); fh.R = (double*)(w + off[4]); fh.lo_out = (double*)(w + off[5]);
        fh.hi_out = (double*)(w + off[6]); fh.x0 = (double*)(w + off[7]); fh.targets = (double*)(w + off[8]);
        fh.targets_copy = targets_out; fh.ld_copy = n;
        hipError_t e = launch_traj_horizon(fa, fh, s);
        if (e != hipSuccess) return hip_fail(h, e, "traj_horizon launch");

        GeneralArgs a;
        std::memset(&a, 0, sizeof(a));
        a.n = n; a.ld = ldw; a.shift_controls = 1;
        a.A = fh.A; a.B = fh.B; a.C = fh.C; a.Q = fh.Q; a.R = fh.R; a.lo = fh.lo_out; a.hi = fh.hi_out;
        a.x0 = fh.x0; a.targets = fh.targets; a.u0 = w + off[9]; a.iters = iters;
        a.flags = h->ws_words + 1;
        const bool fix = wants_cap_resolve(p, algo);
        if (fix && !a.iters) {
            rc = cap_iters_buffer(h, n, &a.iters);
            if (rc) return rc;
        }
        if (fix) {
            rc = resolve_reserve(h, H, TPC_MPC_F64, n);
            if (rc) return rc;
        }
        Workspace ws;
        rc = prepare_workspace(h, algo, H, TPC_MPC_F64, n, &ws, 1);
        if (rc) return rc;
        HIP_TRY(h, hipMemsetAsync(h->ws_words + 1, 0, sizeof(uint32_t), s));
        e = dispatch_general(algo, I, H, TPC_MPC_F64, a, knobs_of(p), ws, s);
        if (e == hipSuccess && fix) {
            Workspace ws2;
            rc = resolve_workspace(h, H, TPC_MPC_F64, n, &ws2);
            if (rc) return rc;
            e = resolve_general(I, H, a, knobs_of(p), ws2, s);
        }
        if (e != hipSuccess) return hip_fail(h, e, "kernel launch");
        HIP_TRY(h, hipMemcpyAsync(steering_front, w + off[9], n * 8, hipMemcpyDeviceToDevice, s));
        HIP_TRY(h, hipMemcpyAsync(steering_rear, w + off[9] + ldw * 8, n * 8, hipMemcpyDeviceToDevice, s));
        e = launch_follow_post(n, target_speed, steering_front, steering_rear, s);
        if (e != hipSuccess) return hip_fail(h, e, "follow_post launch");
        rc = order.end();
        if (rc) return rc;
        return finish_flags(h, flags_out, s);
    });
}

int tpc_mpc_reserve(tpc_mpc_handle h, const tpc_mpc_params* p, int64_t n, int mem) {
    return guarded(h, [&]() -> int {
        int rc = check_common(h, p);
        if (rc) return rc;
        if (n < 0 || n > 0x7fffffffll) return fail(h, TPC_MPC_ERR_BAD_ARG, "need 0 <= n < 2^31");
        if (mem != TPC_MPC_HOST && mem != TPC_MPC_DEVICE) return fail(h, TPC_MPC_ERR_BAD_ARG, "bad memory kind");
        if (n == 0) return TPC_MPC_OK;
        HIP_TRY(h, hipSetDevice(h->device));
        rc = reserve_lane_workspace(h, p->horizon, p->dtype, n);
        if (rc) return rc;
        if (p->algo == TPC_MPC_ALGO_AUTO && p->dtype == TPC_MPC_F64) {
            int32_t* unused = nullptr;
            rc = cap_iters_buffer(h, n, &unused);
            if (rc) return rc;
            Presolve ps;
            if (presolve_lambda(p) > 0.0 && presolve_share(h, n, &ps)) {
                Workspace unused_ws;
                char* side = nullptr;
                rc = presolve_scratch(h, p->horizon, p->dtype, n, 2 * pad256(n * 8) + pad256(n * 4), &unused_ws, &side);
                if (rc) return rc;
            }
        }
        if (mem == TPC_MPC_HOST) {
            const int64_t col = pad256(n * (int64_t)esize(p->dtype)), icol = pad256(n * 4);
            rc = ensure(h, &h->stage, &h->stage_bytes, 5 * col + icol);
            if (rc) return rc;
        }
        return TPC_MPC_OK;
    });
}

int tpc_mpc_x_set_work_hint(tpc_mpc_handle h, const int32_t* hint, int64_t n, int mem) {
    return guarded(h, [&]() -> int {
        if (!h) return fail(nullptr, TPC_MPC_ERR_BAD_ARG, "null handle");
        if (h->host_only) return fail(h, TPC_MPC_ERR_NO_DEVICE, "host-only handle");
        h->hint = nullptr;
        h->hint_n = 0;
        if (!hint || n == 0) return TPC_MPC_OK;
        if (n < 0 || n > 0x7fffffffll) return fail(h, TPC_MPC_ERR_BAD_ARG, "need 0 <= n < 2^31");
        if (mem != TPC_MPC_HOST && mem != TPC_MPC_DEVICE) return fail(h, TPC_MPC_ERR_BAD_ARG, "bad memory kind");
        HIP_TRY(h, hipSetDevice(h->device));
        int rc = ensure(h, &h->hint_own, &h->hint_own_bytes, n * 4);
        if (rc) return rc;
        if (h->have_last) HIP_TRY(h, hipEventSynchronize(h->done_ev));
        HIP_TRY(h, hipMemcpy(h->hint_own, hint, (size_t)n * 4,
                             mem == TPC_MPC_HOST ? hipMemcpyHostToDevice : hipMemcpyDeviceToDevice));
        h->hint = (const int32_t*)h->hint_own;
        h->hint_n = n;
        return TPC_MPC_OK;
    });
}

int tpc_mpc_x_set_queue_key(tpc_mpc_handle h, int on) {
    return guarded(h, [&]() -> int {
        if (!h) return fail(nullptr, TPC_MPC_ERR_BAD_ARG, "null handle");
        if (on != 0 && on != 1) return fail(h, TPC_MPC_ERR_BAD_ARG, "tpc_mpc_x_set_queue_key takes 0 or 1");
        h->opt_queue_key = on != 0;
        return TPC_MPC_OK;
    });
}

int tpc_mpc_x_last_queue_key(tpc_mpc_handle h, int* key) {
    return guarded(h, [&]() -> int {
        if (!h) return fail(nullptr, TPC_MPC_ERR_BAD_ARG, "null handle");
        if (!key) return fail(h, TPC_MPC_ERR_BAD_ARG, "null key");
        *key = h->last_queue_key;
        return TPC_MPC_OK;
    });
}

int tpc_mpc_x_set_group_share(tpc_mpc_handle h, int waves, int cu_count) {
    return guarded(h, [&]() -> int {
        if (!h) return fail(nullptr, TPC_MPC_ERR_BAD_ARG, "null handle");
        if (waves < 0 || cu_count < 0) return fail(h, TPC_MPC_ERR_BAD_ARG, "need waves >= 0, cu_count >= 0");
        h->max_waves = waves;
        h->cu_count = cu_count > 0 ? cu_count : h->device_cu_count;
        return TPC_MPC_OK;
    });
}

int tpc_mpc_x_set_lanex_below(tpc_mpc_handle h, int64_t below) {
    return guarded(h, [&]() -> int {
        if (!h) return fail(nullptr, TPC_MPC_ERR_BAD_ARG, "null handle");
        if (below < -1) return fail(h, TPC_MPC_ERR_BAD_ARG, "need below >= -1");
        h->opt_lanex_below = below;
        return TPC_MPC_OK;
    });
}

int tpc_mpc_set_option(tpc_mpc_handle h, int option, int64_t value) {
    return guarded(h, [&]() -> int {
        if (!h) return fail(nullptr, TPC_MPC_ERR_BAD_ARG, "null handle");
        switch (option) {
            case TPC_MPC_OPT_WAVE_GROUP:
                if (value != 0 && value != 1 && value != 2 && value != 4)
                    return fail(h, TPC_MPC_ERR_BAD_ARG, "TPC_MPC_OPT_WAVE_GROUP takes 0, 1, 2 or 4");
                h->opt_wave_group = (int)value;
                return TPC_MPC_OK;
            case TPC_MPC_OPT_GROUP_LANES:
                if (value != 0 && value != 2 && value != 4 && value != 8)
                    return fail(h, TPC_MPC_ERR_BAD_ARG, "TPC_MPC_OPT_GROUP_LANES takes 0, 2, 4 or 8");
                h->opt_group_lanes = (int)value;
                return TPC_MPC_OK;
            case TPC_MPC_OPT_HOST_SOLVE_ONE:
                if (value < 0 || value > kMaxHorizon) return fail(h, TPC_MPC_ERR_BAD_ARG, "TPC_MPC_OPT_HOST_SOLVE_ONE takes a horizon, 0 .. 64");
                h->opt_host_horizon = (int)value;
                return TPC_MPC_OK;
            case TPC_MPC_OPT_MAILBOX_HOST:
                if (h->host_only) return fail(h, TPC_MPC_ERR_NO_DEVICE, "host-only handle");
                HIP_TRY(h, hipSetDevice(h->device));
                one_shot_destroy(h);
                h->opt_mailbox_host = value != 0;
                return TPC_MPC_OK;
        }
        return fail(h, TPC_MPC_ERR_BAD_ARG, "unknown option %d", option);
    });
}

int tpc_mpc_set_profiling(tpc_mpc_handle h, int enable) {
    return guarded(h, [&]() -> int {
        if (!h) return fail(nullptr, TPC_MPC_ERR_BAD_ARG, "null handle");
        if (h->host_only) return fail(h, TPC_MPC_ERR_NO_DEVICE, "host-only handle");
        HIP_TRY(h, hipSetDevice(h->device));
        if (enable)
            for (auto& e : h->ev) if (!e) HIP_TRY(h, hipEventCreate(&e));
        h->profiling = enable != 0;
        h->ev_valid = false;
        return TPC_MPC_OK;
    });
}

int tpc_mpc_last_kernel_times(tpc_mpc_handle h, double* first_ms, double* second_ms, int* algo) {
    return guarded(h, [&]() -> int {
        if (!h) return fail(nullptr, TPC_MPC_ERR_BAD_ARG, "null handle");
        if (!h->ev_valid)
            return fail(h, TPC_MPC_ERR_BAD_ARG, h->last_algo == kAlgoMixed ? "the last solve was a mixed-horizon batch: its bins ran on child handles"
                                                                            : "no profiled solve on this handle yet");
        HIP_TRY(h, hipEventSynchronize(h->ev[2]));
        float a = 0, b = 0;
        HIP_TRY(h, hipEventElapsedTime(&a, h->ev[0], h->ev[1]));
        HIP_TRY(h, hipEventElapsedTime(&b, h->ev[1], h->ev[2]));
        if (first_ms) *first_ms = a;
// ... 24 lines not shown
```

### trajectory_controller_amd/csrc/tpc_mpc_comm.cpp

```cpp
#include "tpc_mpc_context.h"
#include "tpc_mpc_experimental.h"

#include <dlfcn.h>
#include <cstdlib>
#include <mutex>
#include <rccl/rccl.h>

namespace tpc {

struct Comm {
    ncclComm_t comm = nullptr;
    int rank = 0, world = 1;
};

namespace {

struct Rccl {
    void* lib = nullptr;
    decltype(&ncclGetUniqueId) GetUniqueId = nullptr;
    decltype(&ncclCommInitRank) CommInitRank = nullptr;
    decltype(&ncclCommDestroy) CommDestroy = nullptr;
    decltype(&ncclAllGather) AllGather = nullptr;
    decltype(&ncclBroadcast) Broadcast = nullptr;
    decltype(&ncclGroupStart) GroupStart = nullptr;
// ... 198 lines not shown
    });
}

int tpc_mpc_group_begin(void) {
    return guarded(nullptr, [&]() -> int {
        Rccl* r = rccl();
        if (!r) return fail(nullptr, TPC_MPC_ERR_COMM, "RCCL is not available in this process: %s", g_rccl.why);
        RCCL_TRY(nullptr, r, r->GroupStart());
        return TPC_MPC_OK;
    });
}

int tpc_mpc_group_end(void) {
    return guarded(nullptr, [&]() -> int {
        Rccl* r = rccl();
        if (!r) return fail(nullptr, TPC_MPC_ERR_COMM, "RCCL is not available in this process: %s", g_rccl.why);
        RCCL_TRY(nullptr, r, r->GroupEnd());
        return TPC_MPC_OK;
    });
}

int tpc_mpc_shard_range(int64_t n_total, int rank, int world, int64_t* first, int64_t* count) {
    if (n_total < 0 || world < 1 || rank < 0 || rank >= world || !first || !count) return TPC_MPC_ERR_BAD_ARG;
    shard_range(n_total, rank, world, first, count);
    return TPC_MPC_OK;
}

int tpc_mpc_shard_map(int64_t n_total, int rank, int world, int split, int64_t* first, int64_t* count, int64_t* stride) {
    if (n_total < 0 || world < 1 || rank < 0 || rank >= world || !first || !count || !stride) return TPC_MPC_ERR_BAD_ARG;
    if (split != TPC_MPC_SPLIT_BLOCK && split != TPC_MPC_SPLIT_INTERLEAVED) return TPC_MPC_ERR_BAD_ARG;
    shard_map(n_total, rank, world, split, first, count, stride);
    return TPC_MPC_OK;
}

int tpc_mpc_x_exchange_plan(int64_t n_total, int world, int rank, int split, int force_ragged, int64_t* ops5, int max_ops,
                            int64_t* buffer_elems) {
    if (n_total < 0 || world < 1 || rank < 0 || rank >= world || (max_ops > 0 && !ops5)) return -1;
    if (split != TPC_MPC_SPLIT_BLOCK && split != TPC_MPC_SPLIT_INTERLEAVED) return -1;
    XOp ops[kMaxOps];
    const int n = exchange_plan(n_total, world, rank, split, force_ragged != 0, ops, kMaxOps);
    for (int i = 0; i < n && i < max_ops && i < kMaxOps; ++i) {
        ops5[5 * i] = ops[i].kind; ops5[5 * i + 1] = ops[i].root; ops5[5 * i + 2] = ops[i].send_off;
        ops5[5 * i + 3] = ops[i].recv_off; ops5[5 * i + 4] = ops[i].count;
    }
    if (buffer_elems) *buffer_elems = split == TPC_MPC_SPLIT_INTERLEAVED ? interleaved_cap(n_total, world) * world : n_total;
    return n;
}

int tpc_mpc_solve_batch_compact_sharded_split(tpc_mpc_handle h, const tpc_mpc_params* p, int64_t n_total, int split,
                                              const void* v_shard, const void* delta_y_shard, const void* delta_phi_shard,
                                              void* steering_front_all, void* steering_rear_all, int32_t* iters_shard,
                                              uint32_t* flags_out, void* stream) {
    return guarded(h, [&]() -> int {
        int rc = check_common(h, p);
        if (rc) return rc;
        rc = check_compact_model(h, p);
        if (rc) return rc;
        if (split != TPC_MPC_SPLIT_BLOCK && split != TPC_MPC_SPLIT_INTERLEAVED) return fail(h, TPC_MPC_ERR_BAD_ARG, "split is TPC_MPC_SPLIT_BLOCK or TPC_MPC_SPLIT_INTERLEAVED");
        if (n_total < 0 || n_total > 0x7fffffffll) return fail(h, TPC_MPC_ERR_BAD_ARG, "need 0 <= n_total < 2^31");
        if (n_total == 0) { if (flags_out) *flags_out = 0; return TPC_MPC_OK; }
        if (!steering_front_all || !steering_rear_all) return fail(h, TPC_MPC_ERR_BAD_ARG, "null batch pointer");
        const int rank = h->comm ? h->comm->rank : 0, world = h->comm ? h->comm->world : 1;
        int64_t first = 0, count = 0, stride = 1;
        shard_map(n_total, rank, world, split, &first, &count, &stride);
        if (count > 0 && (!v_shard || !delta_y_shard || !delta_phi_shard)) return fail(h, TPC_MPC_ERR_BAD_ARG, "null batch pointer");
        HIP_TRY(h, hipSetDevice(h->device));
        hipStream_t s = (hipStream_t)stream;
        const int64_t es = (int64_t)esize(p->dtype);
        char* front = (char*)steering_front_all;
        char* rear = (char*)steering_rear_all;
        const bool exchange = world > 1 || h->comm;
        const bool staged = split == TPC_MPC_SPLIT_INTERLEAVED && exchange;
        const int64_t cap = interleaved_cap(n_total, world);
        char *sf = nullptr, *sr = nullptr;
        if (staged) {
            rc = ensure(h, &h->gather, &h->gather_bytes, 2 * pad256(world * cap * es));
            if (rc) return rc;
            sf = (char*)h->gather;
            sr = sf + pad256(world * cap * es);
        }
        StreamOrderScope order(h, s);
        rc = order.begin();
        if (rc) return rc;
        HIP_TRY(h, hipMemsetAsync(h->ws_words + 1, 0, sizeof(uint32_t), s));
        if (count > 0) {
            char* of = staged ? sf + rank * cap * es : front + first * es;
            char* orr = staged ? sr + rank * cap * es : rear + first * es;
            rc = compact_launch(h, p, count, v_shard, delta_y_shard, delta_phi_shard, of, orr, iters_shard, s);
            if (rc) return rc;
        }
        if (exchange) {
            Rccl* r = rccl();
            if (!r) return fail(h, TPC_MPC_ERR_COMM, "RCCL is not available in this process: %s", g_rccl.why);
            XOp ops[kMaxOps];
            const int n_ops = exchange_plan(n_total, world, rank, split, h->comm_test_ragged, ops, kMaxOps);
            GroupScope group(r);
            RCCL_TRY(h, r, group.begin());
            rc = run_plan(h, r, ops, n_ops, staged ? sf : front, (int)es, s);
            if (rc) return rc;
            rc = run_plan(h, r, ops, n_ops, staged ? sr : rear, (int)es, s);
            if (rc) return rc;
            RCCL_TRY(h, r, group.end());
            if (staged) {
                HIP_TRY(h, unpermute(sf, front, n_total, world, cap, (int)es, s));
                HIP_TRY(h, unpermute(sr, rear, n_total, world, cap, (int)es, s));
            }
        }
        rc = order.end();
        if (rc) return rc;
        return finish_flags(h, flags_out, s);
    });
}

int tpc_mpc_solve_batch_compact_sharded(tpc_mpc_handle h, const tpc_mpc_params* p, int64_t n_total,
                                        const void* v_shard, const void* delta_y_shard, const void* delta_phi_shard,
                                        void* steering_front_all, void* steering_rear_all, int32_t* iters_shard,
                                        uint32_t* flags_out, void* stream) {
    return tpc_mpc_solve_batch_compact_sharded_split(h, p, n_total, TPC_MPC_SPLIT_BLOCK, v_shard, delta_y_shard, delta_phi_shard,
                                                     steering_front_all, steering_rear_all, iters_shard, flags_out, stream);
}

int tpc_mpc_solve_batch_general_sharded(tpc_mpc_handle h, const tpc_mpc_params* p, const tpc_mpc_general_io* io_all,
                                        uint32_t* flags_out, void* stream) {
    return guarded(h, [&]() -> int {
        int rc = check_common(h, p);
        if (rc) return rc;
        rc = check_general_device_io(h, io_all);
        if (rc) return rc;
        const int64_t n_total = io_all->n, ld = io_all->ld;
        if (n_total == 0) { if (flags_out) *flags_out = 0; return TPC_MPC_OK; }
        const int rank = h->comm ? h->comm->rank : 0, world = h->comm ? h->comm->world : 1;
        int64_t first = 0, count = 0;
        shard_range(n_total, rank, world, &first, &count);
        HIP_TRY(h, hipSetDevice(h->device));
        hipStream_t s = (hipStream_t)stream;
        const int64_t es = (int64_t)esize(p->dtype);
        const int I = io_all->inputs;
        StreamOrderScope order(h, s);
        rc = order.begin();
        if (rc) return rc;
        HIP_TRY(h, hipMemsetAsync(h->ws_words + 1, 0, sizeof(uint32_t), s));
        if (count > 0) {
            tpc_mpc_general_io blk = *io_all;
            auto at = [&](const void* base) -> const void* { return base ? (const char*)base + first * es : nullptr; };
            blk.n = count;
            blk.A = at(io_all->A); blk.B = at(io_all->B); blk.C = at(io_all->C); blk.Q = at(io_all->Q); blk.R = at(io_all->R);
            blk.lower = at(io_all->lower); blk.upper = at(io_all->upper); blk.x0 = at(io_all->x0); blk.targets = at(io_all->targets);
            blk.controls_inout = (void*)at(io_all->controls_inout); blk.v_inout = (void*)at(io_all->v_inout);
            blk.u0 = (void*)at(io_all->u0);
            blk.iters = io_all->iters ? io_all->iters + first : nullptr;
            rc = general_launch(h, p, &blk, s);
            if (rc) return rc;
        }
        if (world > 1 || h->comm) {
            Rccl* r = rccl();
            if (!r) return fail(h, TPC_MPC_ERR_COMM, "RCCL is not available in this process: %s", g_rccl.why);
            const ncclDataType_t dt = p->dtype == TPC_MPC_F64 ? ncclFloat64 : ncclFloat32;
            ncclComm_t c = h->comm->comm;
            GroupScope group(r);
            RCCL_TRY(h, r, group.begin());
            for (int j = 0; j < I; ++j) {
                char* row = (char*)io_all->u0 + (int64_t)j * ld * es;
                if (n_total % world == 0 && !h->comm_test_ragged) {
                    RCCL_TRY(h, r, r->AllGather(row + first * es, row, (size_t)count, dt, c, s));
                } else {
                    for (int q = 0; q < world; ++q) {
                        int64_t qf = 0, qc = 0;
                        shard_range(n_total, q, world, &qf, &qc);
                        if (qc == 0) continue;
                        RCCL_TRY(h, r, r->Broadcast(row + qf * es, row + qf * es, (size_t)qc, dt, q, c, s));
                    }
                }
            }
            RCCL_TRY(h, r, group.end());
        }
        rc = order.end();
        if (rc) return rc;
        return finish_flags(h, flags_out, s);
    });
}

int tpc_mpc_gather_shards_split(tpc_mpc_handle h, int64_t n_total, int split, void* const* rows, int n_rows, int elem_bytes,
                                void* stream) {
    return guarded(h, [&]() -> int {
        if (!h) return fail(nullptr, TPC_MPC_ERR_BAD_ARG, "null handle");
        if (h->host_only) return fail(h, TPC_MPC_ERR_NO_DEVICE, "a host-only handle has no device arrays to exchange");
        if (split != TPC_MPC_SPLIT_BLOCK && split != TPC_MPC_SPLIT_INTERLEAVED) return fail(h, TPC_MPC_ERR_BAD_ARG, "split is TPC_MPC_SPLIT_BLOCK or TPC_MPC_SPLIT_INTERLEAVED");
        if (n_total < 0 || n_total > 0x7fffffffll) return fail(h, TPC_MPC_ERR_BAD_ARG, "need 0 <= n_total < 2^31");
        if (n_rows < 0 || (n_rows > 0 && !rows)) return fail(h, TPC_MPC_ERR_BAD_ARG, "need n_rows >= 0 and a row table");
        if (elem_bytes != 4 && elem_bytes != 8) return fail(h, TPC_MPC_ERR_BAD_ARG, "elem_bytes is 4 or 8");
        for (int i = 0; i < n_rows; ++i)
            if (!rows[i]) return fail(h, TPC_MPC_ERR_BAD_ARG, "null row pointer");
        if (n_total == 0 || n_rows == 0 || !h->comm) return TPC_MPC_OK;
        const int rank = h->comm->rank, world = h->comm->world;
        int64_t first = 0, count = 0, stride = 1;
        shard_map(n_total, rank, world, split, &first, &count, &stride);
        HIP_TRY(h, hipSetDevice(h->device));
        hipStream_t s = (hipStream_t)stream;
        const int64_t es = elem_bytes;
        const bool staged = split == TPC_MPC_SPLIT_INTERLEAVED;
        const int64_t cap = interleaved_cap(n_total, world);
        if (staged) {
            const int rc0 = ensure(h, &h->gather, &h->gather_bytes, pad256(world * cap * es));
            if (rc0) return rc0;
        }
        StreamOrderScope order(h, s);
        int rc = order.begin();
        if (rc) return rc;
        Rccl* r = rccl();
        if (!r) return fail(h, TPC_MPC_ERR_COMM, "RCCL is not available in this process: %s", g_rccl.why);
        XOp ops[kMaxOps];
        const int n_ops = exchange_plan(n_total, world, rank, split, h->comm_test_ragged, ops, kMaxOps);
        if (!staged) {
            GroupScope group(r);
            RCCL_TRY(h, r, group.begin());
            for (int i = 0; i < n_rows; ++i) {
                rc = run_plan(h, r, ops, n_ops, (char*)rows[i], elem_bytes, s);
                if (rc) return rc;
            }
            RCCL_TRY(h, r, group.end());
        } else {
            char* st = (char*)h->gather;
            for (int i = 0; i < n_rows; ++i) {
                if (count > 0) HIP_TRY(h, hipMemcpyAsync(st + rank * cap * es, rows[i], (size_t)(count * es), hipMemcpyDeviceToDevice, s));
// ... 18 lines not shown
```

### trajectory_controller_amd/csrc/tpc_mpc_context.h

```cpp
#pragma once

#include "../../include/tpc_mpc.h"

#include <hip/hip_runtime.h>

#include <cstdarg>
#include <cstdio>
#include <cstring>
#include <exception>
#include <new>

#include "mpc_internal.h"

namespace tpc {
struct OneShot;
int context_new(int device, int cu_count, tpc_mpc_context** out);
struct Comm;
}

constexpr size_t kTpcErrLen = 512;

struct tpc_mpc_context {
    int device = 0;
    int cu_count = 0;
    int device_cu_count = 0;
    char err[kTpcErrLen] = "";
    void* ws_state = nullptr;
    int64_t ws_bytes = 0;
    uint32_t* ws_words = nullptr;
    void* stage = nullptr;
    int64_t stage_bytes = 0;
    void* roll = nullptr;
    int64_t roll_bytes = 0;
    void* cap_iters = nullptr;
    int64_t cap_iters_bytes = 0;
    void* grad_ws = nullptr;
    int64_t grad_ws_bytes = 0;
    void* newton = nullptr;
    int64_t newton_bytes = 0;
    void* newton_fb = nullptr;
    int64_t newton_fb_bytes = 0;
    void* pre = nullptr;
    int64_t pre_bytes = 0;
    hipStream_t pre_stream = nullptr;
    hipEvent_t pre_fork = nullptr, pre_done = nullptr;
    bool pre_busy = false;
    int pre_group_waves = 0;
    void* mix = nullptr;
    int64_t mix_bytes = 0;
    void* pin_host = nullptr;
    void* pin_dev = nullptr;
    tpc::OneShot* one = nullptr;
    const int32_t* hint = nullptr;
    int64_t hint_n = 0;
    void* hint_own = nullptr;
    int64_t hint_own_bytes = 0;
    bool opt_queue_key = true;
    int last_queue_key = 0;
    bool collect_flags = true;
    uint32_t one_flags = 0;
    int32_t one_iters = 0;
    bool one_valid = false;
    bool profiling = false;
    bool ev_valid = false;
    hipEvent_t ev[3] = {nullptr, nullptr, nullptr};
    int last_algo = 0;
    hipEvent_t done_ev = nullptr;
    hipStream_t last_stream = nullptr;
    bool have_last = false;
    tpc::Comm* comm = nullptr;
    void* gather = nullptr;
    int64_t gather_bytes = 0;
    bool comm_test_force = false, comm_test_ragged = false;
    static constexpr int kMaxKids = 8;
    tpc_mpc_context* kids[kMaxKids] = {nullptr, nullptr, nullptr, nullptr, nullptr, nullptr, nullptr, nullptr};
    hipStream_t kid_stream[kMaxKids] = {nullptr, nullptr, nullptr, nullptr, nullptr, nullptr, nullptr, nullptr};
    hipEvent_t kid_done[kMaxKids] = {nullptr, nullptr, nullptr, nullptr, nullptr, nullptr, nullptr, nullptr};
    hipEvent_t fork_ev = nullptr;
    int opt_wave_group = 0;
    bool opt_mailbox_host = false;
    int64_t one_idle_us = 20000;
    int opt_group_lanes = 0;
    int opt_host_horizon = 0;
    bool host_only = false;
    int64_t opt_lanex_below = -1;
    int max_waves = 0;
};

namespace tpc {

extern thread_local char g_create_error[kTpcErrLen];

__attribute__((format(printf, 3, 4))) inline int fail(tpc_mpc_context* h, int code, const char* fmt, ...) noexcept {
    va_list ap;
    va_start(ap, fmt);
    std::vsnprintf(h ? h->err : g_create_error, kTpcErrLen, fmt, ap);
    va_end(ap);
    return code;
}
inline int hip_fail(tpc_mpc_context* h, hipError_t e, const char* what) noexcept {
    return fail(h, TPC_MPC_ERR_HIP, "%s: %s", what, hipGetErrorString(e));
}
#define HIP_TRY(h, call)                                              \
    do {                                                              \
        hipError_t e__ = (call);                                      \
        if (e__ != hipSuccess) return ::tpc::hip_fail(h, e__, #call); \
    } while (0)

template <class F> int guarded(tpc_mpc_context* h, F&& body) noexcept {
    try {
        return body();
    } catch (const std::bad_alloc&) {
        return fail(h, TPC_MPC_ERR_ALLOC, "out of host memory");
    } catch (const std::exception& e) {
        return fail(h, TPC_MPC_ERR_HIP, "unexpected exception: %s", e.what());
    } catch (...) {
        return fail(h, TPC_MPC_ERR_HIP, "unexpected exception");
    }
}

inline size_t esize(int dtype) { return dtype == TPC_MPC_F64 ? 8 : 4; }
inline int64_t pad256(int64_t bytes) { return (bytes + 255) / 256 * 256; }

inline int ensure(tpc_mpc_context* h, void** buf, int64_t* have, int64_t need) {
    if (need <= *have) return TPC_MPC_OK;
    if (*buf) {
        hipError_t e = hipFree(*buf);
        *buf = nullptr;
        *have = 0;
        if (e != hipSuccess) return hip_fail(h, e, "hipFree");
    }
    const int64_t grow = need + need / 4 + 4096;
    hipError_t e = hipMalloc(buf, (size_t)grow);
    if (e != hipSuccess) {
        *buf = nullptr;
        (void)hipGetLastError();
        return fail(h, TPC_MPC_ERR_ALLOC, "hipMalloc of %lld bytes: %s", (long long)grow, hipGetErrorString(e));
    }
    *have = grow;
    return TPC_MPC_OK;
}

int check_common(tpc_mpc_context* h, const tpc_mpc_params* p, bool host_ok = false);
int check_compact_model(tpc_mpc_context* h, const tpc_mpc_params* p);
int stream_order_begin(tpc_mpc_context* h, hipStream_t s);
int stream_order_end(tpc_mpc_context* h, hipStream_t s);
int finish_flags(tpc_mpc_context* h, uint32_t* flags_out, hipStream_t s);
struct StreamOrderScope {
    tpc_mpc_context* h;
    hipStream_t s;
    bool armed = false;
    StreamOrderScope(tpc_mpc_context* hh, hipStream_t ss) : h(hh), s(ss) {}
    int begin() { const int rc = stream_order_begin(h, s); armed = rc == 0; return rc; }
    int end() { armed = false; return stream_order_end(h, s); }
    ~StreamOrderScope() { if (armed) (void)stream_order_end(h, s); }
};
int general_launch(tpc_mpc_context* h, const tpc_mpc_params* p, const tpc_mpc_general_io* io, hipStream_t s);
int check_general_device_io(tpc_mpc_context* h, const tpc_mpc_general_io* io);
int compact_launch(tpc_mpc_context* h, const tpc_mpc_params* p, int64_t n, const void* v, const void* dy,
                   const void* dphi, void* front, void* rear, int32_t* iters, hipStream_t s);
struct Presolve {
    bool on = false;
    bool deferred = false;
    double lambda_from = 0.0;
    uint32_t limit = 0;
    int group_waves = 0;
    uint32_t* queue = nullptr;
    uint32_t* queue_len = nullptr;
    void *side_front = nullptr, *side_rear = nullptr;
    int32_t* side_iters = nullptr;
    int32_t* select = nullptr;
};
int presolve_begin(tpc_mpc_context* h, const tpc_mpc_params* p, int64_t n, const void* v, const void* dy, const void* dphi,
                   hipStream_t s, Presolve* ps);
int compact_launch_ps(tpc_mpc_context* h, const tpc_mpc_params* p, int64_t n, const void* v, const void* dy,
                      const void* dphi, void* front, void* rear, int32_t* iters, hipStream_t s, Presolve* ps);
int presolve_finish(tpc_mpc_context* h, const tpc_mpc_params* p, int64_t n, const void* v, const void* dy, const void* dphi,
                    void* front, void* rear, int32_t* iters, hipStream_t s, Presolve* ps);
bool group_applicable(const tpc_mpc_context* h, const tpc_mpc_params* p, int H);
int reserve_lane_workspace(tpc_mpc_context* h, int H, int dtype, int64_t n);

int context_new(int device, int cu_count, tpc_mpc_context** out);
int one_shot_solve(tpc_mpc_context* h, const tpc_mpc_params* p, double v, double dy, double dphi, double* front,
                   double* rear);
void one_shot_destroy(tpc_mpc_context* h);
int host_solve_one(const tpc_mpc_params* p, double v, double dy, double dphi, double* front, double* rear, int* iters,
                   unsigned* flags);
void comm_destroy(tpc_mpc_context* h);

}
```

### trajectory_controller_amd/csrc/tpc_mpc_experimental.h

```cpp
#ifndef TPC_MPC_EXPERIMENTAL_H
#define TPC_MPC_EXPERIMENTAL_H

#include "../../include/tpc_mpc.h"

#ifdef __cplusplus
extern "C" {
#endif

int tpc_mpc_x_set_work_hint(tpc_mpc_handle h, const int32_t* hint, int64_t n, int mem);

int tpc_mpc_x_set_queue_key(tpc_mpc_handle h, int on);
int tpc_mpc_x_last_queue_key(tpc_mpc_handle h, int* key);
int tpc_mpc_x_queue_key_predict(const double* v, const double* dy, const double* dphi, int64_t n, float* predicted);

int tpc_mpc_x_set_group_share(tpc_mpc_handle h, int waves, int cu_count);

int tpc_mpc_x_set_lanex_below(tpc_mpc_handle h, int64_t below);

int tpc_mpc_x_exchange_plan(int64_t n_total, int world, int rank, int split, int force_ragged, int64_t* ops5, int max_ops,
                            int64_t* buffer_elems);

#ifdef __cplusplus
}
#endif
#endif
```

### trajectory_controller_amd/csrc/tpc_mpc_mixed.hip

```cpp
#include "tpc_mpc_context.h"

namespace tpc {

namespace {

constexpr int kBinsMax = 8;

struct MixedBins {
    int nb;
    int horizon[kBinsMax];
};

__device__ __forceinline__ int bin_of(const MixedBins& b, int h) {
    int r = b.nb;
#pragma unroll
    for (int i = 0; i < kBinsMax - 1; ++i)
        if (i < b.nb && b.horizon[i] == h) r = i;
    return r;
}

__global__ __launch_bounds__(256) void mixed_bin_kernel(const int32_t* __restrict__ horizons, int64_t n, MixedBins bins,
                                                        uint32_t* __restrict__ counts, uint32_t* __restrict__ slot) {
    const int64_t k = (int64_t)blockIdx.x * blockDim.x + threadIdx.x;
    const bool live = k < n;
// ... 79 lines not shown
                    hc[bins.nb]);
    uint32_t ho[kBinsMax] = {0};
    for (int i = 1; i < kBinsMax; ++i) ho[i] = ho[i - 1] + hc[i - 1];
    HIP_TRY(h, hipMemcpyAsync(offsets, ho, sizeof(ho), hipMemcpyHostToDevice, s));
    hipLaunchKernelGGL((mixed_gather_kernel<T>), dim3(grid), dim3(256), 0, s, d_hz, n, bins, (const uint32_t*)slot,
                       (const uint32_t*)offsets, d_v, d_dy, d_dphi, gv, gdy, gdphi, perm);
    HIP_TRY(h, hipGetLastError());
    int live = 0;
    bool any_group = false;
    for (int i = 0; i < bins.nb; ++i) {
        if (!hc[i]) continue;
        ++live;
        any_group = any_group || group_applicable(h, p, bins.horizon[i]);
    }
    if (!h->fork_ev) HIP_TRY(h, hipEventCreateWithFlags(&h->fork_ev, hipEventDisableTiming));
    if (any_group || live == 1) {
        int last = -1;
        for (int i = 0; i < bins.nb; ++i)
            if (hc[i]) last = i;
        Presolve ps;
        tpc_mpc_params ql = *p;
        ql.horizon = bins.horizon[last];
        const int64_t ol = ho[last];
        int rc = presolve_begin(h, &ql, hc[last], gv + ol, gdy + ol, gdphi + ol, s, &ps);
        ps.deferred = true;
        auto bail = [&](int code) {
            if (ps.on) { (void)hipEventRecord(h->pre_done, h->pre_stream); (void)hipStreamWaitEvent(s, h->pre_done, 0); h->pre_busy = false; }
            return code;
        };
        if (rc) return bail(rc);
        for (int i = 0; i < bins.nb; ++i) {
            if (!hc[i]) continue;
            tpc_mpc_params q = *p;
            q.horizon = bins.horizon[i];
            const int64_t o = ho[i];
            if (i == last) rc = compact_launch_ps(h, &q, hc[i], gv + o, gdy + o, gdphi + o, gfront + o, grear + o, d_iters ? giters + o : nullptr, s, &ps);
            else rc = compact_launch(h, &q, hc[i], gv + o, gdy + o, gdphi + o, gfront + o, grear + o, d_iters ? giters + o : nullptr, s);
            if (rc) return bail(rc);
        }
        rc = presolve_finish(h, &ql, hc[last], gv + ol, gdy + ol, gdphi + ol, gfront + ol, grear + ol, d_iters ? giters + ol : nullptr, s, &ps);
        if (rc) return bail(rc);
        if (live > 1) {
            h->ev_valid = false;
            h->last_algo = kAlgoMixed;
        }
    } else {
        h->ev_valid = false;
        h->last_algo = kAlgoMixed;
        HIP_TRY(h, hipEventRecord(h->fork_ev, s));
        bool forked[kBinsMax] = {false};
        auto join = [&]() {
            for (int i = 0; i < bins.nb; ++i)
                if (forked[i] && hipEventRecord(h->kid_done[i], h->kid_stream[i]) == hipSuccess)
                    (void)hipStreamWaitEvent(s, h->kid_done[i], 0);
        };
        for (int i = bins.nb - 1; i >= 0; --i) {
            if (!hc[i]) continue;
            tpc_mpc_params q = *p;
            q.horizon = bins.horizon[i];
            const int64_t o = ho[i];
            if (!h->kids[i]) {
                tpc_mpc_context* kid = nullptr;
                hipStream_t ks = nullptr;
                hipEvent_t ke = nullptr;
                int rc = context_new(h->device, h->cu_count, &kid);
                if (rc) { join(); return fail(h, rc, "mixed batch: child handle: %s", g_create_error); }
                hipError_t e = hipStreamCreateWithFlags(&ks, hipStreamNonBlocking);
                if (e == hipSuccess) e = hipEventCreateWithFlags(&ke, hipEventDisableTiming);
                if (e != hipSuccess) {
                    if (ks) (void)hipStreamDestroy(ks);
                    (void)tpc_mpc_destroy(kid);
                    join();
                    return hip_fail(h, e, "mixed batch: child stream / event");
                }
                h->kids[i] = kid; h->kid_stream[i] = ks; h->kid_done[i] = ke;
            }
            tpc_mpc_context* kid = h->kids[i];
            kid->opt_wave_group = h->opt_wave_group;
            kid->opt_group_lanes = h->opt_group_lanes;
            hipStream_t ks = h->kid_stream[i];
            hipError_t e = hipStreamWaitEvent(ks, h->fork_ev, 0);
            if (e != hipSuccess) { join(); return hip_fail(h, e, "mixed batch: fork"); }
            forked[i] = true;
            e = hipMemsetAsync(kid->ws_words + 1, 0, sizeof(uint32_t), ks);
            if (e != hipSuccess) { join(); return hip_fail(h, e, "mixed batch: flag word"); }
            int rc = compact_launch(kid, &q, hc[i], gv + o, gdy + o, gdphi + o, gfront + o, grear + o,
                                    d_iters ? giters + o : nullptr, ks);
            if (rc) { join(); return fail(h, rc, "mixed batch, horizon %d: %s", q.horizon, kid->err); }
            hipLaunchKernelGGL(mixed_or_flags_kernel, dim3(1), dim3(1), 0, ks, h->ws_words + 1, (const uint32_t*)(kid->ws_words + 1));
            e = hipGetLastError();
            if (e != hipSuccess) { join(); return hip_fail(h, e, "mixed batch: flags"); }
        }
        {
            hipError_t e = hipSuccess;
            for (int i = 0; i < bins.nb && e == hipSuccess; ++i) {
                if (!forked[i]) continue;
                e = hipEventRecord(h->kid_done[i], h->kid_stream[i]);
                if (e == hipSuccess) e = hipStreamWaitEvent(s, h->kid_done[i], 0);
            }
            if (e != hipSuccess) { join(); return hip_fail(h, e, "mixed batch: join"); }
        }
    }
    hipLaunchKernelGGL((mixed_scatter_kernel<T>), dim3(grid), dim3(256), 0, s, n, (const uint32_t*)perm, (const T*)gfront,
                       (const T*)grear, (const int32_t*)giters, d_front, d_rear, d_iters);
    HIP_TRY(h, hipGetLastError());
    return TPC_MPC_OK;
}

}
}

using namespace tpc;

extern "C" int tpc_mpc_solve_batch_compact_mixed(tpc_mpc_handle h, const tpc_mpc_params* p, int64_t n,
                                                 const int32_t* horizons, const void* v, const void* delta_y,
                                                 const void* delta_phi, void* steering_front, void* steering_rear,
                                                 int32_t* iters, uint32_t* flags_out, int mem, void* stream) {
    return guarded(h, [&]() -> int {
        if (!h) return fail(nullptr, TPC_MPC_ERR_BAD_ARG, "null handle");
        if (!p) return fail(h, TPC_MPC_ERR_BAD_ARG, "null params");
        tpc_mpc_params q = *p;
        int hz[8];
        (void)tpc_mpc_supported_horizons(hz, 8);
        q.horizon = hz[0];
        int rc = check_common(h, &q);
        if (rc) return rc;
        rc = check_compact_model(h, &q);
        if (rc) return rc;
        if (n < 0 || n > 0x7fffffffll) return fail(h, TPC_MPC_ERR_BAD_ARG, "need 0 <= n < 2^31");
        if (mem != TPC_MPC_HOST && mem != TPC_MPC_DEVICE) return fail(h, TPC_MPC_ERR_BAD_ARG, "bad memory kind");
        if (n == 0) { if (flags_out) *flags_out = 0; return TPC_MPC_OK; }
        if (!horizons || !v || !delta_y || !delta_phi || !steering_front || !steering_rear)
            return fail(h, TPC_MPC_ERR_BAD_ARG, "null batch pointer");
        HIP_TRY(h, hipSetDevice(h->device));
        hipStream_t s = (hipStream_t)stream;
        const int64_t es = (int64_t)esize(q.dtype);
        const int64_t col = pad256(n * es), icol = pad256(n * 4);
        const int64_t bin_bytes = 256 + 2 * icol + 5 * col + icol;
        const int64_t host_bytes = mem == TPC_MPC_HOST ? 5 * col + 2 * icol : 0;
        StreamOrderScope order(h, s);
        rc = order.begin();
        if (rc) return rc;
        rc = ensure(h, &h->mix, &h->mix_bytes, bin_bytes + host_bytes);
        if (rc) return rc;
        char* b = (char*)h->mix;
        const void *d_v = v, *d_dy = delta_y, *d_dphi = delta_phi;
        void *d_front = steering_front, *d_rear = steering_rear;
        const int32_t* d_hz = horizons;
        int32_t* d_iters = iters;
        if (mem == TPC_MPC_HOST) {
            char* hb = b + bin_bytes;
            HIP_TRY(h, hipMemcpyAsync(hb, v, n * es, hipMemcpyHostToDevice, s));
            HIP_TRY(h, hipMemcpyAsync(hb + col, delta_y, n * es, hipMemcpyHostToDevice, s));
            HIP_TRY(h, hipMemcpyAsync(hb + 2 * col, delta_phi, n * es, hipMemcpyHostToDevice, s));
            HIP_TRY(h, hipMemcpyAsync(hb + 5 * col, horizons, n * 4, hipMemcpyHostToDevice, s));
            d_v = hb; d_dy = hb + col; d_dphi = hb + 2 * col; d_front = hb + 3 * col; d_rear = hb + 4 * col;
            d_hz = (const int32_t*)(hb + 5 * col);
            d_iters = iters ? (int32_t*)(hb + 5 * col + icol) : nullptr;
        }
        HIP_TRY(h, hipMemsetAsync(h->ws_words + 1, 0, sizeof(uint32_t), s));
        if (q.dtype == TPC_MPC_F64)
            rc = run_mixed<double>(h, &q, n, d_hz, (const double*)d_v, (const double*)d_dy, (const double*)d_dphi,
                                   (double*)d_front, (double*)d_rear, d_iters, b, s);
        else
            rc = run_mixed<float>(h, &q, n, d_hz, (const float*)d_v, (const float*)d_dy, (const float*)d_dphi,
                                  (float*)d_front, (float*)d_rear, d_iters, b, s);
        if (rc) return rc;
        if (mem == TPC_MPC_HOST) {
            HIP_TRY(h, hipMemcpyAsync(steering_front, d_front, n * es, hipMemcpyDeviceToHost, s));
            HIP_TRY(h, hipMemcpyAsync(steering_rear, d_rear, n * es, hipMemcpyDeviceToHost, s));
            if (iters) HIP_TRY(h, hipMemcpyAsync(iters, d_iters, n * 4, hipMemcpyDeviceToHost, s));
            HIP_TRY(h, hipStreamSynchronize(s));
        }
        rc = order.end();
        if (rc) return rc;
        return finish_flags(h, flags_out, s);
    });
}
```

### trajectory_controller_amd/csrc/tpc_mpc_one.hip

```cpp
#include "tpc_mpc_context.h"

#include <chrono>
#include <cstdio>
#include <cstdlib>
#include <cstring>

#include "mpc_wave.h"

namespace tpc {

namespace {

enum : int {
    kW_HorizonQuit = 0,
    kW_Iters = 1,
    kW_Eps = 2, kW_Step = 3, kW_Wheelbase = 4, kW_Q0 = 5, kW_Q1 = 6, kW_Seq0 = 7,
    kW_R0 = 8, kW_R1 = 9, kW_Lo0 = 10, kW_Lo1 = 11, kW_Hi0 = 12, kW_Hi1 = 13, kW_V = 14, kW_Seq1 = 15,
    kW_Dy = 16, kW_Dphi = 17, kW_Seq2 = 23,
    kW_Front = 24, kW_Rear = 25, kW_Alive = 26, kW_Info = 27,
    kW_Timing = 28,
    kReqWords = 24,
};
constexpr uint64_t kSentinel = 0x7ff8dead5eedc0deull;
constexpr uint32_t kMaxPolls = 1u << 26;
// ... 84 lines not shown
}

struct OneShot {
    hipStream_t stream = nullptr;
    hipStream_t launch_stream = nullptr;
    uint64_t seq = 0;
    int horizon = 0;
    uint64_t idle_us = 20000;
    bool disabled = false;
    uint64_t* req_dev = nullptr;
};

namespace {

inline volatile uint64_t* mailbox(tpc_mpc_context* h) { return (volatile uint64_t*)h->pin_host; }
inline volatile uint64_t* request_lines(tpc_mpc_context* h) {
    return h->one && h->one->req_dev ? (volatile uint64_t*)h->one->req_dev : mailbox(h);
}
inline void publish_request() {
#if defined(__x86_64__)
    __builtin_ia32_sfence();
#else
    __atomic_thread_fence(__ATOMIC_SEQ_CST);
#endif
}

int start_kernel(tpc_mpc_context* h, OneShot* o, int horizon, uint64_t start_seq) {
    HIP_TRY(h, hipSetDevice(h->device));
    volatile uint64_t* m = mailbox(h);
    m[kW_Alive] = 1;
    __atomic_thread_fence(__ATOMIC_SEQ_CST);
    uint64_t* dev = (uint64_t*)h->pin_dev;
    const uint64_t* req = o->req_dev ? o->req_dev : dev;
    const uint64_t ticks = o->idle_us * 100ull;
    switch (horizon) {
#define X(hh) case hh: hipLaunchKernelGGL(one_shot_kernel<hh>, dim3(1), dim3(kWave), 0, o->stream, req, dev, start_seq, ticks); break;
        X(4) X(5) X(10) X(20) X(30) X(40)
#undef X
        default: m[kW_Alive] = 0; return fail(h, TPC_MPC_ERR_BAD_HORIZON, "no resident kernel for horizon %d", horizon);
    }
    hipError_t e = hipGetLastError();
    if (e != hipSuccess) { m[kW_Alive] = 0; return hip_fail(h, e, "resident kernel launch"); }
    o->horizon = horizon;
    return TPC_MPC_OK;
}

int stop_kernel(tpc_mpc_context* h, OneShot* o) {
    volatile uint64_t* m = mailbox(h);
    if (o->stream && m[kW_Alive]) {
        HIP_TRY(h, hipSetDevice(h->device));
        volatile uint64_t* rq = request_lines(h);
        const uint64_t seq = ++o->seq;
        rq[kW_HorizonQuit] = 1ull << 32;
        __atomic_thread_fence(__ATOMIC_SEQ_CST);
        publish_request();
        rq[kW_Seq0] = seq; rq[kW_Seq1] = seq; rq[kW_Seq2] = seq;
        publish_request();
        HIP_TRY(h, hipStreamSynchronize(o->stream));
    }
    return TPC_MPC_OK;
}

int launch_path(tpc_mpc_context* h, const tpc_mpc_params* p, double v, double dy, double dphi, double* front, double* rear) {
    HIP_TRY(h, hipSetDevice(h->device));
    tpc_mpc_params q = *p;
    const size_t es = esize(q.dtype);
    char* hp = (char*)h->pin_host + 32 * 8;
    char* dp = (char*)h->pin_dev + 32 * 8;
    if (q.dtype == TPC_MPC_F64) { double* x = (double*)hp; x[0] = v; x[1] = dy; x[2] = dphi; }
    else { float* x = (float*)hp; x[0] = (float)v; x[1] = (float)dy; x[2] = (float)dphi; }
    const uint64_t sentinel64 = kSentinel;
    const uint32_t sentinel32 = 0x7fc5eed1u;
    if (q.dtype == TPC_MPC_F64) { std::memcpy(hp + 3 * es, &sentinel64, 8); std::memcpy(hp + 4 * es, &sentinel64, 8); }
    else { std::memcpy(hp + 3 * es, &sentinel32, 4); std::memcpy(hp + 4 * es, &sentinel32, 4); }
    OneShot* o = h->one;
    if (!o->launch_stream) HIP_TRY(h, hipStreamCreateWithFlags(&o->launch_stream, hipStreamNonBlocking));
    volatile uint32_t* extra = (volatile uint32_t*)(hp + 64);
    const uint32_t sentinel_flags = 0xffffffffu;
    extra[0] = 0; extra[2] = sentinel_flags;
    __atomic_thread_fence(__ATOMIC_SEQ_CST);
    StreamOrderScope order(h, o->launch_stream);
    int rc = order.begin();
    if (rc) return rc;
    HIP_TRY(h, hipMemsetAsync(h->ws_words + 1, 0, sizeof(uint32_t), o->launch_stream));
    rc = compact_launch(h, &q, 1, dp, dp + es, dp + 2 * es, dp + 3 * es, dp + 4 * es, (int32_t*)(dp + 64), o->launch_stream);
    if (rc) return rc;
    HIP_TRY(h, hipMemcpyAsync((void*)(hp + 72), h->ws_words + 1, sizeof(uint32_t), hipMemcpyDeviceToHost, o->launch_stream));
    rc = order.end();
    if (rc) return rc;
    bool done = false;
    const auto t0 = std::chrono::steady_clock::now();
    for (int it = 0; !done; ++it) {
        if (q.dtype == TPC_MPC_F64) {
            const volatile uint64_t* o = (const volatile uint64_t*)(hp + 3 * es);
            done = o[0] != sentinel64 && o[1] != sentinel64;
        } else {
            const volatile uint32_t* o = (const volatile uint32_t*)(hp + 3 * es);
            done = o[0] != sentinel32 && o[1] != sentinel32;
        }
        done = done && extra[2] != sentinel_flags;
        if (!done && (it & 255) == 255 && std::chrono::steady_clock::now() - t0 > std::chrono::milliseconds(2)) break;
    }
    if (!done) HIP_TRY(h, hipStreamSynchronize(o->launch_stream));
    h->one_flags = extra[2];
    h->one_iters = (int32_t)extra[0];
    h->one_valid = true;
    if (q.dtype == TPC_MPC_F64) { *front = ((double*)hp)[3]; *rear = ((double*)hp)[4]; }
    else { *front = ((float*)hp)[3]; *rear = ((float*)hp)[4]; }
    return TPC_MPC_OK;
}

}

void one_shot_destroy(tpc_mpc_context* h) {
    if (!h || !h->one) return;
    OneShot* o = h->one;
#ifdef TPC_ONE_TIMING
    {
        volatile uint64_t* m = mailbox(h);
        if (m[kW_Timing + 2]) fprintf(stderr, "[one timing] %llu solves: request seen -> loops %.0f clocks, loops -> result stored %.0f clocks\n",
                           (unsigned long long)m[kW_Timing + 2], (double)m[kW_Timing] / m[kW_Timing + 2], (double)m[kW_Timing + 1] / m[kW_Timing + 2]);
    }
#endif
    if (o->stream) {
        (void)stop_kernel(h, o);
        (void)hipStreamSynchronize(o->stream);
        (void)hipStreamDestroy(o->stream);
    }
    if (o->launch_stream) {
        (void)hipStreamSynchronize(o->launch_stream);
        (void)hipStreamDestroy(o->launch_stream);
    }
    if (o->req_dev) (void)hipFree(o->req_dev);
    delete o;
    h->one = nullptr;
}

int one_shot_configure(tpc_mpc_context* h, int64_t idle_us) {
    HIP_TRY(h, hipSetDevice(h->device));
    if (!h->one) {
        h->one = new (std::nothrow) OneShot;
        if (!h->one) return fail(h, TPC_MPC_ERR_ALLOC, "out of host memory");
        int large_bar = 0;
        if (!h->opt_mailbox_host &&
            hipDeviceGetAttribute(&large_bar, hipDeviceAttributeIsLargeBar, h->device) == hipSuccess && large_bar) {
            void* p = nullptr;
            if (hipExtMallocWithFlags(&p, 256, hipDeviceMallocFinegrained) == hipSuccess) {
                volatile uint64_t* z = (volatile uint64_t*)p;
                for (int w = 0; w < 32; ++w) z[w] = 0;
                publish_request();
                h->one->req_dev = (uint64_t*)p;
            }
            (void)hipGetLastError();
        }
    }
    OneShot* o = h->one;
    h->one_idle_us = idle_us;
    if (idle_us <= 0) {
        int rc = stop_kernel(h, o);
        if (rc) return rc;
        o->disabled = true;
        return TPC_MPC_OK;
    }
    o->disabled = false;
    o->idle_us = (uint64_t)idle_us;
    return TPC_MPC_OK;
}
// ... 88 lines not shown
```

Before: 62.08 million solves/s.

## Merge scan kernels, reuse zeroed histogram, and batch word-block memsets

The two-kernel histogram scan becomes a single kernel in which each block recomputes the sum of the bins above it with vectorised loads. The scatter kernel now re-zeroes the histogram after use, so the next call can skip the 256 KB memset when a tracked state says the bins are still clean. Several small per-stage memsets of ticket and stats words are folded into one 128-byte reset per solve, with stage bitmasks recording which regions are already clean. This cuts launches and memsets per solve. In exchange it adds state tracking that could go stale if the workspace moves or a kernel aborts.

```diff
diff --git a/trajectory_controller_amd/capi.py b/trajectory_controller_amd/capi.py
--- a/trajectory_controller_amd/capi.py
+++ b/trajectory_controller_amd/capi.py
@@ -205,6 +205,10 @@
                                                               u32p, vp]
     lib.tpc_mpc_gather_shards_split.argtypes = [vp, C.c_int64, C.c_int, C.POINTER(C.c_void_p), C.c_int, C.c_int, vp]
     lib.tpc_mpc_x_exchange_plan.argtypes = [C.c_int64, C.c_int, C.c_int, C.c_int, C.c_int, i64p, C.c_int, i64p]
+    if hasattr(lib, "tpc_mpc_x_bins_rule"):
+        lib.tpc_mpc_x_sort_scratch.argtypes = [C.c_int64, i64p]
+        lib.tpc_mpc_x_sort_scratch.restype = C.c_int64
+        lib.tpc_mpc_x_bins_rule.argtypes = [i32p, i64p, C.c_int, i32p]
     for name in EXPORTS:
         getattr(lib, name)
     if path == LIB_PATH:
diff --git a/trajectory_controller_amd/csrc/mpc_internal.h b/trajectory_controller_amd/csrc/mpc_internal.h
--- a/trajectory_controller_amd/csrc/mpc_internal.h
+++ b/trajectory_controller_amd/csrc/mpc_internal.h
@@ -48,6 +48,21 @@
     int shift_controls;
 };
 
+struct BinsState {
+    const void* at = nullptr;
+    bool clean = false;
+};
+inline void bins_carved(BinsState& b, const void* at, bool moved) {
+    if (moved || at != b.at) { b.at = at; b.clean = false; }
+}
+inline bool bins_counting(BinsState& b, const void* at) {
+    const bool need = !(b.clean && b.at == at);
+    b.at = at;
+    b.clean = false;
+    return need;
+}
+inline void bins_swept(BinsState& b, const void* at) { b.clean = b.at == at; }
+
 struct Workspace {
     void* state;
     uint32_t* ticket;
@@ -56,6 +71,8 @@
     uint32_t *keys, *rank, *order;
     void* sort_temp;
     size_t sort_temp_bytes;
+    BinsState* bins = nullptr;
+    bool words_clean = false;
     hipEvent_t* ev;
     int wave_group = 0;
     int group_lanes = 0;
@@ -78,14 +95,21 @@
 hipError_t generic_general(int dtype, int I, int H, const GeneralArgs& a, const Knobs& k, void* scratch, hipStream_t s);
 
 size_t sort_temp_bytes(int64_t n);
-hipError_t order_begin(void* temp, hipStream_t s);
+hipError_t order_begin(const Workspace& ws, hipStream_t s);
 hipError_t presolve_merge(const uint32_t* queue, const uint32_t* queue_len, int64_t n, const void* sf, const void* sr,
                           const int32_t* si, void* f, void* r, int32_t* it, uint32_t limit, hipStream_t s);
 hipError_t presolve_merge_rows(const uint32_t* queue, const uint32_t* queue_len, int64_t n, const void* su, const int32_t* si,
                                void* u, int32_t* it, int rows, int64_t ld, uint32_t limit, hipStream_t s);
 const uint32_t* order_queue_len(const void* temp);
-hipError_t order_finish(const uint32_t* keys, const uint32_t* rank, uint32_t* order, int64_t n, void* temp,
-                        hipStream_t s);
+hipError_t order_finish(const Workspace& ws, int64_t n, hipStream_t s);
+size_t sort_bins();
+
+inline hipError_t stage_words_reset(const Workspace& ws, bool contiguous, hipStream_t s) {
+    if (ws.words_clean) return hipSuccess;
+    if (contiguous) return hipMemsetAsync(ws.ticket, 0, 32, s);
+    const hipError_t e = hipMemsetAsync(ws.ticket, 0, sizeof(uint32_t), s);
+    return e != hipSuccess ? e : hipMemsetAsync(ws.stats, 0, 3 * sizeof(unsigned long long), s);
+}
 
 struct RolloutStepArgs {
     int64_t n, ld, ld_out, ld_nlt;
diff --git a/trajectory_controller_amd/csrc/mpc_lane_inst.hip b/trajectory_controller_amd/csrc/mpc_lane_inst.hip
--- a/trajectory_controller_amd/csrc/mpc_lane_inst.hip
+++ b/trajectory_controller_amd/csrc/mpc_lane_inst.hip
@@ -37,9 +37,8 @@
 template <typename T, int I, class Model, class Args>
 hipError_t phase1(const Args& a, const Knobs& k, const Workspace& ws, hipStream_t s) {
     T* recs = (T*)ws.state;
-    hipError_t e = hipMemsetAsync(ws.ticket, 0, sizeof(uint32_t), s);
-    if (e == hipSuccess) e = hipMemsetAsync(ws.stats, 0, 3 * sizeof(unsigned long long), s);
-    if (e == hipSuccess) e = order_begin(ws.sort_temp, s);
+    hipError_t e = stage_words_reset(ws, false, s);
+    if (e == hipSuccess) e = order_begin(ws, s);
     if (e != hipSuccess) return e;
     const int cd_grid = (int)((a.n + kWave - 1) / kWave);
     if (ws.ev) (void)hipEventRecord(ws.ev[0], s);
@@ -47,7 +46,7 @@
                        ws.keys, ws.rank, (uint32_t*)ws.sort_temp, ws.stats, wants_state(a) ? 0 : 1);
     e = hipGetLastError();
     if (e != hipSuccess) return e;
-    e = order_finish(ws.keys, ws.rank, ws.order, a.n, ws.sort_temp, s);
+    e = order_finish(ws, a.n, s);
     if (e != hipSuccess) return e;
     if (ws.ev) (void)hipEventRecord(ws.ev[1], s);
     return hipSuccess;
@@ -138,7 +137,7 @@
     if (a.n <= 0) return hipSuccess;
     T* recs = (T*)ws.state;
     uint32_t* queue_len = ws.ticket + 1;
-    hipError_t e = hipMemsetAsync(ws.ticket, 0, 32, s);
+    hipError_t e = stage_words_reset(ws, true, s);
     if (e != hipSuccess) return e;
     const int grid = (int)((a.n + kWave - 1) / kWave);
     hipLaunchKernelGGL((lane_cd_kernel<T, I, kH, Model, Args, SUBSET>), dim3(grid), dim3(kWave), 0, s, a, k, recs, ws.order,
diff --git a/trajectory_controller_amd/csrc/mpc_sort.hip b/trajectory_controller_amd/csrc/mpc_sort.hip
--- a/trajectory_controller_amd/csrc/mpc_sort.hip
+++ b/trajectory_controller_amd/csrc/mpc_sort.hip
@@ -7,31 +7,24 @@
 constexpr int kBins = 1 << 16;
 
 constexpr int kScanBlocks = 64, kScanThreads = 256, kPerThread = kBins / kScanBlocks / kScanThreads;
+static_assert(kPerThread == 4, "one 16-byte load per thread and 1024 bins of another block");
 
-__global__ __launch_bounds__(kScanThreads) void scan_sums_kernel(const uint32_t* __restrict__ hist,
-                                                                 uint32_t* __restrict__ block_sum) {
-    __shared__ uint32_t part[kScanThreads / 64];
-    const int t = threadIdx.x;
-    const int top = kBins - 1 - (blockIdx.x * kScanThreads + t) * kPerThread;
-    uint32_t sum = 0;
-    for (int j = 0; j < kPerThread; ++j) sum += hist[top - j];
-    for (int off = 32; off > 0; off >>= 1) sum += __shfl_down(sum, off);
-    if ((t & 63) == 0) part[t >> 6] = sum;
-    __syncthreads();
-    if (t == 0) {
-        uint32_t tot = 0;
-        for (int w = 0; w < kScanThreads / 64; ++w) tot += part[w];
-        block_sum[blockIdx.x] = tot;
-    }
-}
-
-__global__ __launch_bounds__(kScanThreads) void scan_apply_kernel(uint32_t* __restrict__ hist,
-                                                                  const uint32_t* __restrict__ block_sum) {
+__global__ __launch_bounds__(kScanThreads) void scan_kernel(const uint32_t* __restrict__ hist, uint32_t* __restrict__ base_out) {
     __shared__ uint32_t part[kScanThreads];
+    __shared__ uint32_t above_part[kScanThreads / 64];
     const int t = threadIdx.x;
     const int top = kBins - 1 - (blockIdx.x * kScanThreads + t) * kPerThread;
     uint32_t c[kPerThread], sum = 0;
     for (int j = 0; j < kPerThread; ++j) { c[j] = hist[top - j]; sum += c[j]; }
+    const uint4* above4 = (const uint4*)(hist + (kBins - (int)blockIdx.x * kScanThreads * kPerThread));
+    uint32_t above = 0;
+#pragma unroll 4
+    for (int j = 0; j < (int)blockIdx.x; ++j) {
+        const uint4 q = above4[j * kScanThreads + t];
+        above += (q.x + q.y) + (q.z + q.w);
+    }
+    for (int off = 32; off > 0; off >>= 1) above += __shfl_down(above, off);
+    if ((t & 63) == 0) above_part[t >> 6] = above;
     part[t] = sum;
     __syncthreads();
     for (int off = 1; off < kScanThreads; off <<= 1) {
@@ -41,40 +34,48 @@
         __syncthreads();
     }
     uint32_t base = part[t] - sum;
-    for (int b = 0; b < (int)blockIdx.x; ++b) base += block_sum[b];
+    for (int w = 0; w < kScanThreads / 64; ++w) base += above_part[w];
     for (int j = 0; j < kPerThread; ++j) {
-        hist[top - j] = base;
+        base_out[top - j] = base;
         base += c[j];
     }
 }
 
 __global__ void scatter_kernel(const uint32_t* __restrict__ keys, const uint32_t* __restrict__ rank,
-                               const uint32_t* __restrict__ base, uint32_t* __restrict__ order, int64_t n) {
-    for (int64_t i = (int64_t)blockIdx.x * blockDim.x + threadIdx.x; i < n; i += (int64_t)gridDim.x * blockDim.x)
-        order[base[keys[i] >> 16] + rank[i]] = (uint32_t)i;
+                               const uint32_t* __restrict__ base, uint32_t* __restrict__ order, int64_t n,
+                               uint32_t* __restrict__ hist) {
+    const int64_t first = (int64_t)blockIdx.x * blockDim.x + threadIdx.x, stride = (int64_t)gridDim.x * blockDim.x;
+    for (int64_t i = first; i < n; i += stride) order[base[keys[i] >> 16] + rank[i]] = (uint32_t)i;
+    for (int64_t i = first; i < kBins; i += stride) hist[i] = 0u;
 }
 
 }
 
-size_t sort_temp_bytes(int64_t) { return (size_t)(kBins + kScanBlocks) * sizeof(uint32_t); }
+size_t sort_temp_bytes(int64_t) { return (size_t)(2 * kBins) * sizeof(uint32_t); }
+size_t sort_bins() { return (size_t)kBins; }
 
-const uint32_t* order_queue_len(const void* temp) { return (const uint32_t*)temp + 127; }
+const uint32_t* order_queue_len(const void* temp) { return (const uint32_t*)temp + kBins + 127; }
 
-hipError_t order_begin(void* temp, hipStream_t s) {
-    return hipMemsetAsync(temp, 0, (size_t)kBins * sizeof(uint32_t), s);
+hipError_t order_begin(const Workspace& ws, hipStream_t s) {
+    const bool need = ws.bins ? bins_counting(*ws.bins, ws.sort_temp) : true;
+    if (!need) return hipSuccess;
+    return hipMemsetAsync(ws.sort_temp, 0, (size_t)kBins * sizeof(uint32_t), s);
 }
 
-hipError_t order_finish(const uint32_t* keys, const uint32_t* rank, uint32_t* order, int64_t n, void* temp,
-                        hipStream_t s) {
-    uint32_t* hist = (uint32_t*)temp;
+hipError_t order_finish(const Workspace& ws, int64_t n, hipStream_t s) {
+    uint32_t* hist = (uint32_t*)ws.sort_temp;
+    uint32_t* base = hist + kBins;
     const int block = 256;
     int64_t g = (n + block - 1) / block;
     const unsigned grid = (unsigned)(g < 2048 ? g : 2048);
-    uint32_t* block_sum = hist + kBins;
-    hipLaunchKernelGGL(scan_sums_kernel, dim3(kScanBlocks), dim3(kScanThreads), 0, s, (const uint32_t*)hist, block_sum);
-    hipLaunchKernelGGL(scan_apply_kernel, dim3(kScanBlocks), dim3(kScanThreads), 0, s, hist, (const uint32_t*)block_sum);
-    hipLaunchKernelGGL(scatter_kernel, dim3(grid), dim3(block), 0, s, keys, rank, (const uint32_t*)hist, order, n);
-    return hipGetLastError();
+    hipLaunchKernelGGL(scan_kernel, dim3(kScanBlocks), dim3(kScanThreads), 0, s, (const uint32_t*)hist, base);
+    hipError_t e = hipGetLastError();
+    if (e != hipSuccess) return e;
+    hipLaunchKernelGGL(scatter_kernel, dim3(grid), dim3(block), 0, s, (const uint32_t*)ws.keys, (const uint32_t*)ws.rank,
+                       (const uint32_t*)base, ws.order, n, hist);
+    e = hipGetLastError();
+    if (e == hipSuccess && ws.bins) bins_swept(*ws.bins, ws.sort_temp);
+    return e;
 }
 
 template <typename T>
diff --git a/trajectory_controller_amd/csrc/mpc_ub_inst.hip b/trajectory_controller_amd/csrc/mpc_ub_inst.hip
--- a/trajectory_controller_amd/csrc/mpc_ub_inst.hip
+++ b/trajectory_controller_amd/csrc/mpc_ub_inst.hip
@@ -37,9 +37,8 @@
 template <typename T, bool EQB>
 hipError_t phase1(const CompactArgs& a, const Knobs& k, const Workspace& ws, hipStream_t s) {
     T* recs = (T*)ws.state;
-    hipError_t e = hipMemsetAsync(ws.ticket, 0, sizeof(uint32_t), s);
-    if (e == hipSuccess) e = hipMemsetAsync(ws.stats, 0, 3 * sizeof(unsigned long long), s);
-    if (e == hipSuccess) e = order_begin(ws.sort_temp, s);
+    hipError_t e = stage_words_reset(ws, false, s);
+    if (e == hipSuccess) e = order_begin(ws, s);
     if (e != hipSuccess) return e;
     const int cd_grid = (int)((a.n + kWave - 1) / kWave);
     if (ws.ev) (void)hipEventRecord(ws.ev[0], s);
@@ -47,7 +46,7 @@
                        (uint32_t*)ws.sort_temp, ws.stats);
     e = hipGetLastError();
     if (e != hipSuccess) return e;
-    e = order_finish(ws.keys, ws.rank, ws.order, a.n, ws.sort_temp, s);
+    e = order_finish(ws, a.n, s);
     if (e != hipSuccess) return e;
     if (ws.ev) (void)hipEventRecord(ws.ev[1], s);
     return hipSuccess;
diff --git a/trajectory_controller_amd/csrc/mpc_ubg_inst.hip b/trajectory_controller_amd/csrc/mpc_ubg_inst.hip
--- a/trajectory_controller_amd/csrc/mpc_ubg_inst.hip
+++ b/trajectory_controller_amd/csrc/mpc_ubg_inst.hip
@@ -35,9 +35,8 @@
 template <typename T, int I>
 hipError_t phase1(const GeneralArgs& a, const Knobs& k, const Workspace& ws, hipStream_t s) {
     T* recs = (T*)ws.state;
-    hipError_t e = hipMemsetAsync(ws.ticket, 0, sizeof(uint32_t), s);
-    if (e == hipSuccess) e = hipMemsetAsync(ws.stats, 0, 3 * sizeof(unsigned long long), s);
-    if (e == hipSuccess) e = order_begin(ws.sort_temp, s);
+    hipError_t e = stage_words_reset(ws, false, s);
+    if (e == hipSuccess) e = order_begin(ws, s);
     if (e != hipSuccess) return e;
     const int cd_grid = (int)((a.n + kWave - 1) / kWave);
     if (ws.ev) (void)hipEventRecord(ws.ev[0], s);
@@ -45,7 +44,7 @@
                        (uint32_t*)ws.sort_temp, ws.stats);
     e = hipGetLastError();
     if (e != hipSuccess) return e;
-    e = order_finish(ws.keys, ws.rank, ws.order, a.n, ws.sort_temp, s);
+    e = order_finish(ws, a.n, s);
     if (e != hipSuccess) return e;
     if (ws.ev) (void)hipEventRecord(ws.ev[1], s);
     return hipSuccess;
diff --git a/trajectory_controller_amd/csrc/tpc_mpc_api.cpp b/trajectory_controller_amd/csrc/tpc_mpc_api.cpp
--- a/trajectory_controller_amd/csrc/tpc_mpc_api.cpp
+++ b/trajectory_controller_amd/csrc/tpc_mpc_api.cpp
@@ -312,6 +312,9 @@
     ws->keys = ws->rank = ws->order = nullptr;
     ws->sort_temp = nullptr;
     ws->sort_temp_bytes = 0;
+    ws->bins = nullptr;
+    ws->words_clean = words_take(h, kWordsFirst);
+    const int64_t had_bytes = h->ws_bytes;
     if (algo == kAlgoGeneric) {
         int rc = ensure(h, &h->ws_state, &h->ws_bytes, pad256(generic_scratch_bytes(H, dtype, n)));
         if (rc) return rc;
@@ -338,8 +341,10 @@
         ws->order = (uint32_t*)(b + rec_b + 2 * col_b);
         ws->sort_temp = b + rec_b + 3 * col_b;
         ws->sort_temp_bytes = tmp_b;
+        ws->bins = &h->bins;
         ws->capacity_bytes = h->ws_bytes;
     }
+    bins_carved(h->bins, ws->sort_temp, h->ws_bytes != had_bytes);
     return TPC_MPC_OK;
 }
 
@@ -347,12 +352,15 @@
 int resolve_workspace(tpc_mpc_context* h, int H, int dtype, int64_t n, Workspace* ws) {
     const bool ev_valid = h->ev_valid;
     const int last_algo = h->last_algo;
+    const uint32_t words_clean = h->words_clean;
     const int rc = prepare_workspace(h, TPC_MPC_ALGO_LANE, H, dtype, n, ws);
     h->ev_valid = ev_valid;
     h->last_algo = last_algo;
+    h->words_clean = words_clean;
     ws->ev = nullptr;
     ws->ticket = h->ws_words + 16;
     ws->stats = (unsigned long long*)(h->ws_words + 18);
+    ws->words_clean = rc == TPC_MPC_OK && words_take(h, kWordsResolve);
     return rc;
 }
 
@@ -432,10 +440,12 @@
 int reserve_lane_workspace(tpc_mpc_context* h, int H, int dtype, int64_t n) {
     const bool ev_valid = h->ev_valid;
     const int last_algo = h->last_algo;
+    const uint32_t words_clean = h->words_clean;
     Workspace ws;
     const int rc = prepare_workspace(h, horizon_specialised(H) ? TPC_MPC_ALGO_LANE : kAlgoGeneric, H, dtype, n, &ws);
     h->ev_valid = ev_valid;
     h->last_algo = last_algo;
+    h->words_clean = words_clean;
     return rc;
 }
 
@@ -484,6 +494,7 @@
     ws->cu_count = h->cu_count;
     ws->ticket = h->ws_words + 24;
     ws->stats = (unsigned long long*)(h->ws_words + 26);
+    ws->words_clean = words_take(h, kWordsPresolve);
     *side = b + lane_b;
     return TPC_MPC_OK;
 }
@@ -915,7 +926,8 @@
         StreamOrderScope order(h, s);
         rc = order.begin();
         if (rc) return rc;
-        HIP_TRY(h, hipMemsetAsync(h->ws_words + 1, 0, sizeof(uint32_t), s));
+        rc = words_reset(h, s);
+        if (rc) return rc;
         if (mem == TPC_MPC_DEVICE) {
             rc = compact_launch(h, p, n, v, delta_y, delta_phi, steering_front, steering_rear, iters, s);
             if (rc) return rc;
@@ -1058,10 +1070,11 @@
             if (rc) return rc;
         }
 
+        rc = words_reset(h, s);
+        if (rc) return rc;
         Workspace ws;
         rc = prepare_workspace(h, algo, H, p->dtype, n, &ws, 1);
         if (rc) return rc;
-        HIP_TRY(h, hipMemsetAsync(h->ws_words + 1, 0, sizeof(uint32_t), s));
         hipError_t e = dispatch_general(algo, I, H, p->dtype, a, knobs_of(p), ws, s);
         if (e == hipSuccess && fix) {
             Workspace ws2;
@@ -1405,6 +1418,7 @@
         for (int st = 0; st < steps; ++st) {
             hipError_t e = dispatch_general(algo, I, H, p->dtype, a, kn, ws, s);
             if (e != hipSuccess) return hip_fail(h, e, "kernel launch");
+            ws.words_clean = false;
             r.step = st;
             if (polished) {
                 pa.status = d_status ? d_status + (int64_t)st * ld_out : nullptr;
@@ -2116,7 +2130,8 @@
         fa.target_speed = target_speed; fa.target_distance = target_distance;
         hipError_t e = launch_traj_point(fa, s);
         if (e != hipSuccess) return hip_fail(h, e, "traj_point launch");
-        HIP_TRY(h, hipMemsetAsync(h->ws_words + 1, 0, sizeof(uint32_t), s));
+        rc = words_reset(h, s);
+        if (rc) return rc;
         rc = compact_launch(h, p, n, fa.v_out, fa.ysoll_out, fa.phisoll_out, steering_front, steering_rear, iters, s);
         if (rc) return rc;
         e = launch_follow_post(n, target_speed, steering_front, steering_rear, s);
@@ -2189,10 +2204,11 @@
             rc = resolve_reserve(h, H, TPC_MPC_F64, n);
             if (rc) return rc;
         }
+        rc = words_reset(h, s);
+        if (rc) return rc;
         Workspace ws;
         rc = prepare_workspace(h, algo, H, TPC_MPC_F64, n, &ws, 1);
         if (rc) return rc;
-        HIP_TRY(h, hipMemsetAsync(h->ws_words + 1, 0, sizeof(uint32_t), s));
         e = dispatch_general(algo, I, H, TPC_MPC_F64, a, knobs_of(p), ws, s);
         if (e == hipSuccess && fix) {
             Workspace ws2;
@@ -2229,7 +2245,9 @@
             if (presolve_lambda(p) > 0.0 && presolve_share(h, n, &ps)) {
                 Workspace unused_ws;
                 char* side = nullptr;
+                const uint32_t words_clean = h->words_clean;
                 rc = presolve_scratch(h, p->horizon, p->dtype, n, 2 * pad256(n * 8) + pad256(n * 4), &unused_ws, &side);
+                h->words_clean = words_clean;
                 if (rc) return rc;
             }
         }
@@ -2270,6 +2288,27 @@
         h->opt_queue_key = on != 0;
         return TPC_MPC_OK;
     });
+}
+
+int64_t tpc_mpc_x_sort_scratch(int64_t n, int64_t* bins) {
+    if (bins) *bins = (int64_t)sort_bins();
+    return (int64_t)sort_temp_bytes(n);
+}
+
+int tpc_mpc_x_bins_rule(const int32_t* event, const int64_t* at, int count, int32_t* out) {
+    if (!event || !at || !out || count < 0) return -1;
+    BinsState b;
+    for (int i = 0; i < count; ++i) {
+        const void* p = (const void*)(intptr_t)at[i];
+        switch (event[i]) {
+            case 0: bins_carved(b, p, false); out[i] = b.clean; break;
+            case 1: bins_carved(b, p, true); out[i] = b.clean; break;
+            case 2: out[i] = bins_counting(b, p); break;
+            case 3: bins_swept(b, p); out[i] = b.clean; break;
+            default: return -1;
+        }
+    }
+    return 0;
 }
 
 int tpc_mpc_x_last_queue_key(tpc_mpc_handle h, int* key) {
diff --git a/trajectory_controller_amd/csrc/tpc_mpc_comm.cpp b/trajectory_controller_amd/csrc/tpc_mpc_comm.cpp
--- a/trajectory_controller_amd/csrc/tpc_mpc_comm.cpp
+++ b/trajectory_controller_amd/csrc/tpc_mpc_comm.cpp
@@ -304,7 +304,8 @@
         StreamOrderScope order(h, s);
         rc = order.begin();
         if (rc) return rc;
-        HIP_TRY(h, hipMemsetAsync(h->ws_words + 1, 0, sizeof(uint32_t), s));
+        rc = words_reset(h, s);
+        if (rc) return rc;
         if (count > 0) {
             char* of = staged ? sf + rank * cap * es : front + first * es;
             char* orr = staged ? sr + rank * cap * es : rear + first * es;
@@ -361,7 +362,8 @@
         StreamOrderScope order(h, s);
         rc = order.begin();
         if (rc) return rc;
-        HIP_TRY(h, hipMemsetAsync(h->ws_words + 1, 0, sizeof(uint32_t), s));
+        rc = words_reset(h, s);
+        if (rc) return rc;
         if (count > 0) {
             tpc_mpc_general_io blk = *io_all;
             auto at = [&](const void* base) -> const void* { return base ? (const char*)base + first * es : nullptr; };
diff --git a/trajectory_controller_amd/csrc/tpc_mpc_context.h b/trajectory_controller_amd/csrc/tpc_mpc_context.h
--- a/trajectory_controller_amd/csrc/tpc_mpc_context.h
+++ b/trajectory_controller_amd/csrc/tpc_mpc_context.h
@@ -28,6 +28,8 @@
     void* ws_state = nullptr;
     int64_t ws_bytes = 0;
     uint32_t* ws_words = nullptr;
+    uint32_t words_clean = 0;
+    tpc::BinsState bins;
     void* stage = nullptr;
     int64_t stage_bytes = 0;
     void* roll = nullptr;
@@ -146,6 +148,19 @@
 int stream_order_begin(tpc_mpc_context* h, hipStream_t s);
 int stream_order_end(tpc_mpc_context* h, hipStream_t s);
 int finish_flags(tpc_mpc_context* h, uint32_t* flags_out, hipStream_t s);
+constexpr uint32_t kWordsFirst = 1u, kWordsResolve = 2u, kWordsPresolve = 4u;
+inline int words_reset(tpc_mpc_context* h, hipStream_t s) {
+    h->words_clean = 0;
+    const hipError_t e = hipMemsetAsync(h->ws_words, 0, 128, s);
+    if (e != hipSuccess) return hip_fail(h, e, "hipMemsetAsync(ws_words)");
+    h->words_clean = kWordsFirst | kWordsResolve | kWordsPresolve;
+    return TPC_MPC_OK;
+}
+inline bool words_take(tpc_mpc_context* h, uint32_t stage) {
+    const bool clean = (h->words_clean & stage) != 0;
+    h->words_clean &= ~stage;
+    return clean;
+}
 struct StreamOrderScope {
     tpc_mpc_context* h;
     hipStream_t s;
diff --git a/trajectory_controller_amd/csrc/tpc_mpc_experimental.h b/trajectory_controller_amd/csrc/tpc_mpc_experimental.h
--- a/trajectory_controller_amd/csrc/tpc_mpc_experimental.h
+++ b/trajectory_controller_amd/csrc/tpc_mpc_experimental.h
@@ -20,6 +20,9 @@
 int tpc_mpc_x_exchange_plan(int64_t n_total, int world, int rank, int split, int force_ragged, int64_t* ops5, int max_ops,
                             int64_t* buffer_elems);
 
+int64_t tpc_mpc_x_sort_scratch(int64_t n, int64_t* bins);
+int tpc_mpc_x_bins_rule(const int32_t* event, const int64_t* at, int count, int32_t* out);
+
 #ifdef __cplusplus
 }
 #endif
diff --git a/trajectory_controller_amd/csrc/tpc_mpc_mixed.hip b/trajectory_controller_amd/csrc/tpc_mpc_mixed.hip
--- a/trajectory_controller_amd/csrc/tpc_mpc_mixed.hip
+++ b/trajectory_controller_amd/csrc/tpc_mpc_mixed.hip
@@ -185,9 +185,9 @@
             hipError_t e = hipStreamWaitEvent(ks, h->fork_ev, 0);
             if (e != hipSuccess) { join(); return hip_fail(h, e, "mixed batch: fork"); }
             forked[i] = true;
-            e = hipMemsetAsync(kid->ws_words + 1, 0, sizeof(uint32_t), ks);
-            if (e != hipSuccess) { join(); return hip_fail(h, e, "mixed batch: flag word"); }
-            int rc = compact_launch(kid, &q, hc[i], gv + o, gdy + o, gdphi + o, gfront + o, grear + o,
+            int rc = words_reset(kid, ks);
+            if (rc) { join(); return fail(h, rc, "mixed batch: word block: %s", kid->err); }
+            rc = compact_launch(kid, &q, hc[i], gv + o, gdy + o, gdphi + o, gfront + o, grear + o,
                                     d_iters ? giters + o : nullptr, ks);
             if (rc) { join(); return fail(h, rc, "mixed batch, horizon %d: %s", q.horizon, kid->err); }
             hipLaunchKernelGGL(mixed_or_flags_kernel, dim3(1), dim3(1), 0, ks, h->ws_words + 1, (const uint32_t*)(kid->ws_words + 1));
@@ -261,7 +261,8 @@
             d_hz = (const int32_t*)(hb + 5 * col);
             d_iters = iters ? (int32_t*)(hb + 5 * col + icol) : nullptr;
         }
-        HIP_TRY(h, hipMemsetAsync(h->ws_words + 1, 0, sizeof(uint32_t), s));
+        rc = words_reset(h, s);
+        if (rc) return rc;
         if (q.dtype == TPC_MPC_F64)
             rc = run_mixed<double>(h, &q, n, d_hz, (const double*)d_v, (const double*)d_dy, (const double*)d_dphi,
                                    (double*)d_front, (double*)d_rear, d_iters, b, s);
diff --git a/trajectory_controller_amd/csrc/tpc_mpc_one.hip b/trajectory_controller_amd/csrc/tpc_mpc_one.hip
--- a/trajectory_controller_amd/csrc/tpc_mpc_one.hip
+++ b/trajectory_controller_amd/csrc/tpc_mpc_one.hip
@@ -190,7 +190,8 @@
     StreamOrderScope order(h, o->launch_stream);
     int rc = order.begin();
     if (rc) return rc;
-    HIP_TRY(h, hipMemsetAsync(h->ws_words + 1, 0, sizeof(uint32_t), o->launch_stream));
+    rc = words_reset(h, o->launch_stream);
+    if (rc) return rc;
     rc = compact_launch(h, &q, 1, dp, dp + es, dp + 2 * es, dp + 3 * es, dp + 4 * es, (int32_t*)(dp + 64), o->launch_stream);
     if (rc) return rc;
     HIP_TRY(h, hipMemcpyAsync((void*)(hp + 72), h->ws_words + 1, sizeof(uint32_t), hipMemcpyDeviceToHost, o->launch_stream));
```

Measured after the change: 62.36 million solves/s, median of 6. Within noise of the previous version (+0.5%).
